# voidful/DeSTA2.5-Audio

Hardware: AMD Instinct MI355X
Metric: train steps/sec (node) Whisper-v3+Llama3.1-8B Q-Former6L at 1/2/4/8 MI355X (higher is better)
Workload: dtype bf16

## Files before the change

desta2.5-audio_amd/csrc/attention.hip:

```cpp
#include "common.h"
#include <mutex>
#include "desta_hip.h"

#ifndef ATTN_ABL
#define ATTN_ABL 0
#endif

namespace {

typedef __attribute__((ext_vector_type(4))) __bf16 bf16x4;

struct AttnArgs {
    const bf16_t* Q; const bf16_t* K; const bf16_t* V; bf16_t* O;
    const bf16_t* dO; bf16_t* dQ; bf16_t* dK; bf16_t* dV;
    float* lse; const float* delta;
    float* O32;
    const float* rope_cs;
    long q_bs, q_rs, k_bs, k_rs, v_bs, v_rs, o_bs, o_rs;
    long do_bs, do_rs, dq_bs, dq_rs, dk_bs, dk_rs, dv_bs, dv_rs;
    int B, Hq, Hkv, Sq, Sk;
    int causal;
    const int* kv_start;
    float scale_log2;
    float scale;
    unsigned drop_thresh, seed_lo, seed_hi; float drop_scale;
    long dkv_t_ld;
};

template <int D>
__device__ __forceinline__ int img_off(int row, int ch) {
    const int sw = (D == 128) ? (((row & 3) << 2) | ((row >> 2) & 3)) : ((((row >> 1) & 1) << 2) | ((row >> 2) & 3));
    return row * (D * 2) + ((ch ^ sw) << 4);
}

template <int N> struct stage_vec;
template <> struct stage_vec<1> { typedef __attribute__((ext_vector_type(4))) unsigned type; };
template <> struct stage_vec<2> { typedef __attribute__((ext_vector_type(8))) unsigned type; };
template <> struct stage_vec<4> { typedef __attribute__((ext_vector_type(16))) unsigned type; };
template <int D, int ROWS, int NT = 256> using stage_t = typename stage_vec<ROWS * (D / 8) / NT>::type;

template <int D, int ROWS, int NT = 256>
__device__ __forceinline__ stage_t<D, ROWS, NT> tile_load(const bf16_t* base, long rs, int row0, int max_row) {
    constexpr int CH = D / 8, N = ROWS * CH / NT;
    stage_t<D, ROWS, NT> out;
#pragma unroll
    for (int i = 0; i < N; ++i) {
        const int id = i * NT + threadIdx.x;
        const int r = id / CH, c = id % CH;
        const int gr = min(row0 + r, max_row);
        const uint4 v = *(const uint4*)(base + (long)gr * rs + c * 8);
        out[4 * i + 0] = v.x; out[4 * i + 1] = v.y; out[4 * i + 2] = v.z; out[4 * i + 3] = v.w;
    }
    return out;
}
template <int D, int ROWS, int NT = 256>
__device__ __forceinline__ void tile_store(char* img, const stage_t<D, ROWS, NT>& regs) {
    constexpr int CH = D / 8, N = ROWS * CH / NT;
#pragma unroll
    for (int i = 0; i < N; ++i) {
        const int id = i * NT + threadIdx.x;
        const int r = id / CH, c = id % CH;
        *(uint4*)(img + img_off<D>(r, c)) = make_uint4(regs[4 * i + 0], regs[4 * i + 1], regs[4 * i + 2], regs[4 * i + 3]);
    }
}

template <int D>
__device__ __forceinline__ bf16x8 frag_rows(const char* img, int row0, int ks, int lane) {
    const int r = row0 + (lane & 31);
    return *(const bf16x8*)(img + img_off<D>(r, 2 * ks + (lane >> 5)));
}

template <int D>
__device__ __forceinline__ bf16x8 frag_tr(const char* img, int row0, int col0, int lane) {
    const int i = lane & 15, g = (lane >> 4) & 1, h = lane >> 5;
    const int q = i >> 2, pp = i & 3;
    const int c = col0 + 16 * g + 4 * pp;
    const int r_lo = row0 + 4 * h + q;
    const int a0 = img_off<D>(r_lo, c >> 3) + ((c & 4) << 1);
    const int a1 = img_off<D>(r_lo + 8, c >> 3) + ((c & 4) << 1);
    const bf16x4 lo = __builtin_amdgcn_ds_read_tr16_b64_v4bf16((__attribute__((address_space(3))) bf16x4*)(img + a0));
    const bf16x4 hi = __builtin_amdgcn_ds_read_tr16_b64_v4bf16((__attribute__((address_space(3))) bf16x4*)(img + a1));
    bf16x8 out;
    out[0] = lo[0]; out[1] = lo[1]; out[2] = lo[2]; out[3] = lo[3];
    out[4] = hi[0]; out[5] = hi[1]; out[6] = hi[2]; out[7] = hi[3];
    return out;
}

__device__ __forceinline__ bf16x8 acc_frag(const f32x16& x, int s) {
    bf16x8 o;
#pragma unroll
    for (int j = 0; j < 8; ++j) o[j] = (__bf16)x[8 * s + j];
    return o;
}

__device__ __forceinline__ int acc_row(int reg, int lane) { return (reg & 3) + 8 * (reg >> 2) + 4 * (lane >> 5); }

__device__ __forceinline__ void attn_work_item(const AttnArgs& p, int nq, int& qblk, int& h, int& b) {
    const int id = blockIdx.x, per = nq * (p.Hq / p.Hkv), ngrp = p.B * p.Hkv;
    int g, r;
    if ((ngrp & 7) == 0) {
        const int xcd = id & 7, slot = id >> 3;
        g = (slot / per) * 8 + xcd;
        r = slot % per;
    } else {
        g = id / per;
        r = id % per;
    }
    b = g / p.Hkv;
    h = (g % p.Hkv) * (p.Hq / p.Hkv) + r / nq;
    qblk = r % nq;
    if (p.causal) qblk = nq - 1 - qblk;
}

#ifndef ATTN_FWD_PF
#define ATTN_FWD_PF 1
#endif
#ifndef ATTN_FWD64_WAVES
#define ATTN_FWD64_WAVES 3
#endif
template <int D, bool DROP, int NW = 4>
__global__ __launch_bounds__(64 * NW, NW == 4 ? (D == 64 ? ATTN_FWD64_WAVES : 2) : 2) void attn_fwd_k(AttnArgs p) {
    constexpr int NT = 64 * NW, QB = 32 * NW;
    __shared__ __attribute__((aligned(16))) char lds[2 * 64 * D * 2];
    char* kimg = lds;
    char* vimg = lds + 64 * D * 2;
    const int lane = threadIdx.x & 63, wave = __builtin_amdgcn_readfirstlane(threadIdx.x >> 6), h2 = lane >> 5;
    int qblk, h, b;
    attn_work_item(p, (p.Sq + QB - 1) / QB, qblk, h, b);
    const int qb0 = qblk * QB, q0 = qb0 + wave * 32;
    const int hk = h / (p.Hq / p.Hkv);
    const int qcol = q0 + (lane & 31);

    const bf16_t* qptr = p.Q + (long)b * p.q_bs + (long)min(qcol, p.Sq - 1) * p.q_rs + (long)h * D;
    bf16x8 qf[D / 16];
#pragma unroll
    for (int ds = 0; ds < D / 16; ++ds) qf[ds] = *(const bf16x8*)(qptr + 16 * ds + 8 * h2);

    const int coff = p.Sk - p.Sq;
    const int kv_lo = p.kv_start ? max(0, min(p.kv_start[b], p.Sk)) : 0;
    int kv_hi = p.Sk;
    if (p.causal) kv_hi = min(p.Sk, min(qb0 + QB - 1, p.Sq - 1) + coff + 1);
    const int t_lo = kv_lo / 64, t_hi = (kv_hi + 63) / 64;
    const int q_abs = qcol + coff;
    const int wave_kmax = p.causal ? min(q0 + 31, p.Sq - 1) + coff : p.Sk - 1;

    const bf16_t* kbase = p.K + (long)b * p.k_bs + (long)hk * D;
    const bf16_t* vbase = p.V + (long)b * p.v_bs + (long)hk * D;

    f32x16 oacc[D / 32];
#pragma unroll
    for (int i = 0; i < D / 32; ++i)
#pragma unroll
        for (int r = 0; r < 16; ++r) oacc[i][r] = 0.f;
    float m = -INFINITY, l = 0.f;

    constexpr int PF = ATTN_FWD_PF;
    stage_t<D, 64, NT> kr0 = {}, vr0 = {}, kr1 = {}, vr1 = {};
    if (t_lo < t_hi) {
        kr0 = tile_load<D, 64, NT>(kbase, p.k_rs, t_lo * 64, p.Sk - 1);
        vr0 = tile_load<D, 64, NT>(vbase, p.v_rs, t_lo * 64, p.Sk - 1);
    }
    if (PF == 2 && t_lo + 1 < t_hi) {
        kr1 = tile_load<D, 64, NT>(kbase, p.k_rs, (t_lo + 1) * 64, p.Sk - 1);
        vr1 = tile_load<D, 64, NT>(vbase, p.v_rs, (t_lo + 1) * 64, p.Sk - 1);
    }
    auto compute = [&](const int kt) __attribute__((always_inline)) {
        if (kt * 64 > wave_kmax) return;
        f32x16 st[2];
#pragma unroll
        for (int kb = 0; kb < 2; ++kb)
#pragma unroll
            for (int r = 0; r < 16; ++r) st[kb][r] = 0.f;
        {
            constexpr int NS = (ATTN_ABL == 4 ? 1 : D / 16);
            bf16x8 ka[NS], kbf[NS];
#pragma unroll
            for (int ds = 0; ds < NS; ++ds) ka[ds] = frag_rows<D>(kimg, 0, ds, lane);
            __builtin_amdgcn_sched_barrier(0);
#pragma unroll
            for (int ds = 0; ds < NS; ++ds) {
                st[0] = __builtin_amdgcn_mfma_f32_32x32x16_bf16(ka[ds], qf[ds], st[0], 0, 0, 0);
                kbf[ds] = frag_rows<D>(kimg, 32, ds, lane);
            }
            __builtin_amdgcn_sched_barrier(0);
#pragma unroll
            for (int ds = 0; ds < NS; ++ds) st[1] = __builtin_amdgcn_mfma_f32_32x32x16_bf16(kbf[ds], qf[ds], st[1], 0, 0, 0);
        }
        const bool need_mask = (kt * 64 + 63 >= p.Sk) || (kt * 64 < kv_lo) || (p.causal && kt * 64 + 63 > q0 + coff);
        if (need_mask) {
            asm volatile("; boundary tile" ::: "memory");
#pragma unroll
            for (int kb = 0; kb < 2; ++kb)
#pragma unroll
                for (int r = 0; r < 16; ++r) {
                    const int key = kt * 64 + kb * 32 + acc_row(r, lane);
                    const bool ok = key < p.Sk && key >= kv_lo && (!p.causal || key <= q_abs);
                    st[kb][r] = ok ? st[kb][r] : -INFINITY;
                }
        }
        float tmax = -INFINITY;
#pragma unroll
        for (int kb = 0; kb < 2; ++kb)
#pragma unroll
            for (int r = 0; r < 16; ++r) tmax = fmaxf(tmax, st[kb][r]);
        tmax = fmaxf(tmax, __shfl_xor(tmax, 32, 64)) * p.scale_log2;
        const float mnew = fmaxf(m, tmax);
        const float muse = (mnew == -INFINITY) ? 0.f : mnew;
        const float alpha = __builtin_amdgcn_exp2f(m - muse);
        typedef float f32x2 __attribute__((ext_vector_type(2)));
        f32x2 rs2 = {0.f, 0.f};
        const f32x2 sc2 = {p.scale_log2, p.scale_log2}, nm2 = {-muse, -muse};
#pragma unroll
        for (int kb = 0; kb < 2; ++kb)
#pragma unroll
            for (int r = 0; r < 16; r += 2) {
                const f32x2 sv = {st[kb][r], st[kb][r + 1]};
                const f32x2 av = sv * sc2 + nm2;
// ... 426 lines not shown
    for (int ds = 0; ds < D / 16; ++ds) {
        qf[ds] = *(const bf16x8*)(qptr + 16 * ds + 8 * h2);
        gf[ds] = *(const bf16x8*)(gptr + 16 * ds + 8 * h2);
    }
    const long stat = ((long)b * p.Hq + h) * p.Sq + qc;
    const float lse = p.lse[stat], dlt = p.delta[stat];

    const int coff = p.Sk - p.Sq;
    const int kv_lo = p.kv_start ? max(0, min(p.kv_start[b], p.Sk)) : 0;
    int kv_hi = p.Sk;
    if (p.causal) kv_hi = min(p.Sk, min(qb0 + QB - 1, p.Sq - 1) + coff + 1);
    const int t_lo = kv_lo / 64, t_hi = (kv_hi + 63) / 64;
    const int q_abs = qcol + coff;
    const int wave_kmax = p.causal ? min(q0 + 31, p.Sq - 1) + coff : p.Sk - 1;

    const bf16_t* kbase = p.K + (long)b * p.k_bs + (long)hk * D;
    const bf16_t* vbase = p.V + (long)b * p.v_bs + (long)hk * D;

    f32x16 dq[D / 32];
#pragma unroll
    for (int i = 0; i < D / 32; ++i)
#pragma unroll
        for (int r = 0; r < 16; ++r) dq[i][r] = 0.f;

    constexpr int PF = ATTN_DQ_PF;
    stage_t<D, 64, NT> kr0 = {}, vr0 = {}, kr1 = {}, vr1 = {};
    if (t_lo < t_hi) {
        kr0 = tile_load<D, 64, NT>(kbase, p.k_rs, t_lo * 64, p.Sk - 1);
        vr0 = tile_load<D, 64, NT>(vbase, p.v_rs, t_lo * 64, p.Sk - 1);
    }
    if (PF == 2 && t_lo + 1 < t_hi) {
        kr1 = tile_load<D, 64, NT>(kbase, p.k_rs, (t_lo + 1) * 64, p.Sk - 1);
        vr1 = tile_load<D, 64, NT>(vbase, p.v_rs, (t_lo + 1) * 64, p.Sk - 1);
    }
    auto compute = [&](const int kt) __attribute__((always_inline)) {
        if (kt * 64 > wave_kmax) return;
#pragma unroll
        for (int kb = 0; kb < 2; ++kb) {
            f32x16 st, dp;
#pragma unroll
            for (int r = 0; r < 16; ++r) { st[r] = 0.f; dp[r] = 0.f; }
#pragma unroll
            for (int ds = 0; ds < D / 16; ++ds) {
                st = __builtin_amdgcn_mfma_f32_32x32x16_bf16(frag_rows<D>(kimg, kb * 32, ds, lane), qf[ds], st, 0, 0, 0);
                dp = __builtin_amdgcn_mfma_f32_32x32x16_bf16(frag_rows<D>(vimg, kb * 32, ds, lane), gf[ds], dp, 0, 0, 0);
            }
            const bool need_mask = (kt * 64 + kb * 32 + 31 >= p.Sk) || (kt * 64 + kb * 32 < kv_lo) ||
                                   (p.causal && kt * 64 + kb * 32 + 31 > q0 + coff);
            unsigned keep = 0xffffu;
            if constexpr (DROP) {
                const unsigned long rowbase = (((unsigned long)b * p.Hq + h) * p.Sq + qc) * p.Sk;
                keep = 0;
#pragma unroll
                for (int r = 0; r < 16; r += 2) {
                    const unsigned long i0 = rowbase + (kt * 64 + kb * 32 + acc_row(r, lane));
                    const unsigned hsh = desta_rng32(p.seed_lo, p.seed_hi, i0 >> 1);
                    keep |= ((hsh & 0xffffu) >= p.drop_thresh ? 1u : 0u) << r;
                    keep |= ((hsh >> 16) >= p.drop_thresh ? 1u : 0u) << (r + 1);
                }
            }
            if (need_mask) {
                asm volatile("; boundary tile" ::: "memory");
#pragma unroll
                for (int r = 0; r < 16; ++r) {
                    const int key = kt * 64 + kb * 32 + acc_row(r, lane);
                    const bool ok = key < p.Sk && key >= kv_lo && (!p.causal || key <= q_abs);
                    st[r] = ok ? st[r] : -INFINITY;
                }
            }
#pragma unroll
            for (int r = 0; r < 16; ++r) {
                const float pv = __builtin_amdgcn_exp2f(fmaf(st[r], p.scale_log2, -lse));
                float dpr = dp[r];
                if constexpr (DROP) dpr = ((keep >> r) & 1u) ? dpr * p.drop_scale : 0.f;
                st[r] = pv * (dpr - dlt) * p.scale;
            }
#pragma unroll
            for (int s = 0; s < 2; ++s) {
                const bf16x8 dsf = acc_frag(st, s);
#pragma unroll
                for (int i = 0; i < D / 32; ++i)
                    dq[i] = __builtin_amdgcn_mfma_f32_32x32x16_bf16(frag_tr<D>(kimg, kb * 32 + 16 * s, i * 32, lane), dsf, dq[i], 0, 0, 0);
            }
        }
    };
#define DESTA_KV_STAGE(KT, KR, VR)                                                   \
    __syncthreads();                         \
    asm volatile("; stage " #KR ::: "memory");  \
    tile_store<D, 64, NT>(kimg, KR);                                                     \
    tile_store<D, 64, NT>(vimg, VR);                                                     \
    __syncthreads();                                                                 \
    if ((KT) + PF < t_hi) {                                                          \
        KR = tile_load<D, 64, NT>(kbase, p.k_rs, ((KT) + PF) * 64, p.Sk - 1);            \
        VR = tile_load<D, 64, NT>(vbase, p.v_rs, ((KT) + PF) * 64, p.Sk - 1);            \
    }
    for (int kt = t_lo; kt < t_hi; kt += 2) {
        DESTA_KV_STAGE(kt, kr0, vr0)
        compute(kt);
        if (kt + 1 < t_hi) {
            if constexpr (PF == 2) {
                DESTA_KV_STAGE(kt + 1, kr1, vr1)
            } else {
                DESTA_KV_STAGE(kt + 1, kr0, vr0)
            }
            compute(kt + 1);
        }
    }
#undef DESTA_KV_STAGE
    if (qcol < p.Sq) {
        bf16_t* optr = p.dQ + (long)b * p.dq_bs + (long)qcol * p.dq_rs + (long)h * D;
#pragma unroll
        for (int i = 0; i < D / 32; ++i)
#pragma unroll
            for (int rq = 0; rq < 4; ++rq) {
                u16x4 o;
#pragma unroll
                for (int e = 0; e < 4; ++e) o[e] = f2bf(dq[i][4 * rq + e]);
                *(u16x4*)(optr + i * 32 + 8 * rq + 4 * h2) = o;
            }
    }
}

template <int D, bool CAUSAL, int HPB>
__global__ __launch_bounds__(512, 2) void attn_bwd_dq8_k(AttnArgs p, float* __restrict__ delta_out) {
    constexpr int NT = 512, RB = 256 / HPB, WPH = RB / 32;
    constexpr int TILE = 64 * D * 2, SLOT = 2 * TILE;
    constexpr int NCH = 64 * (D / 8) / NT;
    __shared__ __attribute__((aligned(16))) char lds[2 * SLOT];
    const int lane = threadIdx.x & 63, wave = __builtin_amdgcn_readfirstlane(threadIdx.x >> 6), h2 = lane >> 5;
    const int G = p.Hq / p.Hkv, nq = (p.Sq + RB - 1) / RB, hgroups = G / HPB, ngrp = p.B * p.Hkv;
    int g, qblk, hg;
    {
        const int id = blockIdx.x, per = nq * hgroups;
        if ((ngrp & 7) == 0) {
            const int xcd = id & 7, slot = id >> 3, gpx = ngrp >> 3;
            if (CAUSAL) {
                const int r = slot % (hgroups * gpx);
                qblk = nq - 1 - slot / (hgroups * gpx); hg = r / gpx; g = (r % gpx) * 8 + xcd;
            } else {
                const int r = slot % per;
                g = (slot / per) * 8 + xcd; hg = r / nq; qblk = r % nq;
            }
        } else if (CAUSAL) {
            const int r = id % (hgroups * ngrp);
            qblk = nq - 1 - id / (hgroups * ngrp); hg = r / ngrp; g = r % ngrp;
        } else {
            const int r = id % per;
            g = id / per; hg = r / nq; qblk = r % nq;
        }
    }
    const int b = g / p.Hkv, hk = g % p.Hkv;
    const int h = hk * G + hg * HPB + wave / WPH;
    const int qb0 = qblk * RB, q0 = qb0 + (wave % WPH) * 32;
    const int qcol = q0 + (lane & 31), qc = min(qcol, p.Sq - 1);
    const bool wave_on = q0 < p.Sq;

    const int coff = p.Sk - p.Sq;
    const int kv_lo = p.kv_start ? max(0, min(p.kv_start[b], p.Sk)) : 0;
    int kv_hi = p.Sk;
    if (CAUSAL) kv_hi = min(p.Sk, min(qb0 + RB - 1, p.Sq - 1) + coff + 1);
    const int t_lo = kv_lo / 64, t_hi = (kv_hi + 63) / 64;
    const int q_abs = qcol + coff;
    const int wave_kmax = CAUSAL ? min(q0 + 31, p.Sq - 1) + coff : p.Sk - 1;

    const char* kbase = (const char*)(p.K + (long)b * p.k_bs + (long)hk * D);
    const char* vbase = (const char*)(p.V + (long)b * p.v_bs + (long)hk * D);
    int srow[NCH], sdst[NCH];
    unsigned ksrc[NCH], vsrc[NCH];
#pragma unroll
    for (int i = 0; i < NCH; ++i) {
        const int id = i * NT + threadIdx.x, r = id / (D / 8), c = id % (D / 8);
        srow[i] = r;
        sdst[i] = img_off<D>(r, c);
        ksrc[i] = (unsigned)(r * (int)p.k_rs + c * 8) * 2u;
        vsrc[i] = (unsigned)(r * (int)p.v_rs + c * 8) * 2u;
    }
    typedef typename stage_vec<NCH>::type stage8_t;
    stage8_t kr = {}, vr = {};
    auto load_tile = [&](const int kt) __attribute__((always_inline)) {
        const char* kb_ = kbase + (long)kt * 64 * p.k_rs * 2;
        const char* vb_ = vbase + (long)kt * 64 * p.v_rs * 2;
        const bool ragged = kt * 64 + 64 > p.Sk;
#pragma unroll
        for (int i = 0; i < NCH; ++i) {
            unsigned ko = ksrc[i], vo = vsrc[i];
            if (ragged) {
                const int rc = max(min(srow[i], p.Sk - 1 - kt * 64), -kt * 64), c = (i * NT + (int)threadIdx.x) % (D / 8);
                ko = (unsigned)(rc * (int)p.k_rs + c * 8) * 2u;
                vo = (unsigned)(rc * (int)p.v_rs + c * 8) * 2u;
            }
            const uint4 a = *(const uint4*)(kb_ + (long)(int)ko), c4 = *(const uint4*)(vb_ + (long)(int)vo);
            kr[4 * i + 0] = a.x; kr[4 * i + 1] = a.y; kr[4 * i + 2] = a.z; kr[4 * i + 3] = a.w;
            vr[4 * i + 0] = c4.x; vr[4 * i + 1] = c4.y; vr[4 * i + 2] = c4.z; vr[4 * i + 3] = c4.w;
        }
    };
    auto store_tile = [&](char* slot) __attribute__((always_inline)) {
#pragma unroll
        for (int i = 0; i < NCH; ++i) {
            *(uint4*)(slot + sdst[i]) = make_uint4(kr[4 * i + 0], kr[4 * i + 1], kr[4 * i + 2], kr[4 * i + 3]);
            *(uint4*)(slot + TILE + sdst[i]) = make_uint4(vr[4 * i + 0], vr[4 * i + 1], vr[4 * i + 2], vr[4 * i + 3]);
        }
    };

    load_tile(t_lo);
    const bf16_t* qptr = p.Q + (long)b * p.q_bs + (long)qc * p.q_rs + (long)h * D;
    const bf16_t* gptr = p.dO + (long)b * p.do_bs + (long)qc * p.do_rs + (long)h * D;
    const bf16_t* optr = p.O + (long)b * p.o_bs + (long)qc * p.o_rs + (long)h * D;
    bf16x8 qf[D / 16], gf[D / 16];
    float dl = 0.f;
#pragma unroll
    for (int ds = 0; ds < D / 16; ++ds) {
        qf[ds] = *(const bf16x8*)(qptr + 16 * ds + 8 * h2);
        gf[ds] = *(const bf16x8*)(gptr + 16 * ds + 8 * h2);
        const bf16x8 of = *(const bf16x8*)(optr + 16 * ds + 8 * h2);
#pragma unroll
        for (int j = 0; j < 8; ++j) dl += (float)of[j] * (float)gf[ds][j];
    }
    const long stat = ((long)b * p.Hq + h) * p.Sq + qc;
    const float nlse = -p.lse[stat];
    const float dlt = swap_halves_sum(dl);
    if (wave_on && qcol < p.Sq && h2 == 0) delta_out[stat] = dlt;
#pragma unroll
    for (int ds = 0; ds < D / 16; ++ds) asm volatile("" :: "v"(qf[ds]), "v"(gf[ds]));
    asm volatile("" :: "v"(nlse));
    store_tile(lds);
    load_tile(t_lo + 1);

    int kofs[D / 16], tofs[D / 32][2];
#pragma unroll
    for (int ds = 0; ds < D / 16; ++ds) {
        kofs[ds] = img_off<D>(lane & 31, 2 * ds + h2);
        asm volatile("" : "+v"(kofs[ds]));
    }
    {
        const int i16 = lane & 15, gq = (lane >> 4) & 1, qq = i16 >> 2, pp = i16 & 3;
#pragma unroll
        for (int i = 0; i < D / 32; ++i) {
            const int c = i * 32 + 16 * gq + 4 * pp;
            tofs[i][0] = img_off<D>(4 * h2 + qq, c >> 3) + ((c & 4) << 1);
            tofs[i][1] = img_off<D>(4 * h2 + qq + 8, c >> 3) + ((c & 4) << 1);
            asm volatile("" : "+v"(tofs[i][0]), "+v"(tofs[i][1]));
        }
    }
    f32x16 dq[D / 32];
#pragma unroll
    for (int i = 0; i < D / 32; ++i)
#pragma unroll
        for (int r = 0; r < 16; ++r) dq[i][r] = 0.f;
#define ATTN_BARRIER() asm volatile("s_waitcnt lgkmcnt(0)\n\ts_barrier" ::: "memory")
    ATTN_BARRIER();

    int sb = 0;
    for (int kt = t_lo; kt < t_hi; ++kt) {
        const int sn = SLOT - sb;
        const bool act = wave_on && kt * 64 <= wave_kmax;
        if (act) {
            int kad[D / 16];
#pragma unroll
            for (int ds = 0; ds < D / 16; ++ds) { kad[ds] = kofs[ds] + sb; asm volatile("" : "+v"(kad[ds])); }
#pragma unroll
            for (int kb = 0; kb < 2; ++kb) {
                if (CAUSAL && kt * 64 + kb * 32 > wave_kmax) break;
                f32x16 st, dp;
#pragma unroll
                for (int r = 0; r < 16; ++r) { st[r] = 0.f; dp[r] = 0.f; }
#pragma unroll
                for (int ds = 0; ds < D / 16; ++ds) {
                    st = __builtin_amdgcn_mfma_f32_32x32x16_bf16(*(const bf16x8*)(lds + kad[ds] + kb * 32 * D * 2), qf[ds], st, 0, 0, 0);
                    dp = __builtin_amdgcn_mfma_f32_32x32x16_bf16(*(const bf16x8*)(lds + kad[ds] + TILE + kb * 32 * D * 2), gf[ds], dp, 0, 0, 0);
                }
                const bool need_mask = (kt * 64 + kb * 32 + 31 >= p.Sk) || (kt * 64 + kb * 32 < kv_lo) ||
                                       (CAUSAL && kt * 64 + kb * 32 + 31 > q0 + coff);
                if (need_mask) {
                    asm volatile("; boundary tile" ::: "memory");
#pragma unroll
                    for (int r = 0; r < 16; ++r) {
                        const int key = kt * 64 + kb * 32 + acc_row(r, lane);
                        const bool ok = key < p.Sk && key >= kv_lo && (!CAUSAL || key <= q_abs);
                        st[r] = ok ? st[r] : -INFINITY;
                    }
                }
#pragma unroll
                for (int r = 0; r < 16; ++r) {
                    const float pv = __builtin_amdgcn_exp2f(fmaf(st[r], p.scale_log2, nlse));
                    st[r] = pv * ((dp[r] - dlt) * p.scale);
                }
                int tad[D / 32][2];
#pragma unroll
                for (int i = 0; i < D / 32; ++i)
#pragma unroll
                    for (int j = 0; j < 2; ++j) { tad[i][j] = tofs[i][j] + sb + kb * 32 * D * 2; asm volatile("" : "+v"(tad[i][j])); }
#pragma unroll
                for (int s = 0; s < 2; ++s) {
                    const bf16x8 dsf = acc_frag(st, s);
#pragma unroll
                    for (int i = 0; i < D / 32; ++i)
                        dq[i] = __builtin_amdgcn_mfma_f32_32x32x16_bf16(tr_pair(lds + tad[i][0] + 16 * s * D * 2, lds + tad[i][1] + 16 * s * D * 2), dsf, dq[i], 0, 0, 0);
                }
            }
        }
        if (kt + 1 < t_hi) {
            store_tile(lds + sn);
            if (kt + 2 < t_hi) load_tile(kt + 2);
        }
        ATTN_BARRIER();
        sb = sn;
    }
#undef ATTN_BARRIER

    if (wave_on && qcol < p.Sq) {
        bf16_t* dqp = p.dQ + (long)b * p.dq_bs + (long)qcol * p.dq_rs + (long)h * D;
        if (p.rope_cs) {
            const float* cs = p.rope_cs + (long)qcol * D;
#pragma unroll
            for (int i = 0; i < D / 32; ++i)
#pragma unroll
                for (int jj = 0; jj < 4; ++jj) {
                    const float4 c4 = *(const float4*)(cs + (32 * i + 8 * jj + 4 * h2));
                    const float g0 = dq[i][4 * jj], g1 = dq[i][4 * jj + 1], g2 = dq[i][4 * jj + 2], g3 = dq[i][4 * jj + 3];
                    dq[i][4 * jj] = g0 * c4.x + g1 * c4.y;     dq[i][4 * jj + 1] = g1 * c4.x - g0 * c4.y;
                    dq[i][4 * jj + 2] = g2 * c4.z + g3 * c4.w; dq[i][4 * jj + 3] = g3 * c4.z - g2 * c4.w;
                }
        }
#pragma unroll
        for (int i = 0; i < D / 32; ++i)
#pragma unroll
            for (int j = 0; j < 2; ++j) {
                unsigned a[2], c[2];
#pragma unroll
                for (int e = 0; e < 2; ++e) {
                    a[e] = (unsigned)f2bf(dq[i][8 * j + 2 * e]) | ((unsigned)f2bf(dq[i][8 * j + 2 * e + 1]) << 16);
                    c[e] = (unsigned)f2bf(dq[i][8 * j + 4 + 2 * e]) | ((unsigned)f2bf(dq[i][8 * j + 4 + 2 * e + 1]) << 16);
                }
                const auto r0 = __builtin_amdgcn_permlane32_swap(a[0], c[0], false, false);
                const auto r1 = __builtin_amdgcn_permlane32_swap(a[1], c[1], false, false);
                *(uint4*)(dqp + i * 32 + 16 * j + 8 * h2) = make_uint4(r0[0], r1[0], r0[1], r1[1]);
            }
    }
}

#ifndef ATTN_DKDV_QR
#define ATTN_DKDV_QR 32
#endif

template <int D, bool DROP, int NW = 4>
__global__ __launch_bounds__(64 * NW, (NW == 4 && D == 64) ? 2 : 1) void attn_bwd_dkdv_k(AttnArgs p) {
    constexpr int QR = (D == 128) ? ATTN_DKDV_QR : 32;
    constexpr int NT = 64 * NW, KB = 32 * NW;
    constexpr int LDS_LOOP = 2 * QR * D * 2 + 2 * QR * 4, LDS_EPI = NW * 32 * 64 * 4;
    __shared__ __attribute__((aligned(16))) char lds[LDS_LOOP > LDS_EPI ? LDS_LOOP : LDS_EPI];
    char* qimg = lds;
    char* gimg = lds + QR * D * 2;
    float* lse_s = (float*)(lds + 2 * QR * D * 2);
    float* dlt_s = lse_s + QR;
    const int lane = threadIdx.x & 63, wave = __builtin_amdgcn_readfirstlane(threadIdx.x >> 6), h2 = lane >> 5;
    const int nhb = p.Hkv * p.B;
    const int kb0 = (blockIdx.x / nhb) * KB, k0 = kb0 + wave * 32;
    const int hk = (blockIdx.x % nhb) % p.Hkv, b = (blockIdx.x % nhb) / p.Hkv, group = p.Hq / p.Hkv;
    const int kcol = k0 + (lane & 31), kc = min(kcol, p.Sk - 1);
    const int kv_lo = p.kv_start ? max(0, min(p.kv_start[b], p.Sk)) : 0;
    const int coff = p.Sk - p.Sq;

    const bf16_t* kptr = p.K + (long)b * p.k_bs + (long)kc * p.k_rs + (long)hk * D;
    const bf16_t* vptr = p.V + (long)b * p.v_bs + (long)kc * p.v_rs + (long)hk * D;
    bf16x8 kf[D / 16], vf[D / 16];
#pragma unroll
    for (int ds = 0; ds < D / 16; ++ds) {
        kf[ds] = *(const bf16x8*)(kptr + 16 * ds + 8 * h2);
        vf[ds] = *(const bf16x8*)(vptr + 16 * ds + 8 * h2);
    }
    const bool key_ok = kcol < p.Sk && kcol >= kv_lo;

    f32x16 dk[D / 32], dv[D / 32];
#pragma unroll
    for (int i = 0; i < D / 32; ++i)
#pragma unroll
        for (int r = 0; r < 16; ++r) { dk[i][r] = 0.f; dv[i][r] = 0.f; }

    const int q_first = p.causal ? max(0, kb0 - coff) : 0;
    const int qt_lo = q_first / QR, qt_hi = (p.Sq + QR - 1) / QR;
    const int nq = qt_hi - qt_lo, n_it = group * nq;
    stage_t<D, QR, NT> qr0 = {}, gr0 = {}, qr1 = {}, gr1 = {};
    float ls0 = 0.f, dl0 = 0.f, ls1 = 0.f, dl1 = 0.f;
#define DESTA_Q_FETCH(IT, QR_, GR, LS, DL)                                                                      \
    {                                                                                                          \
        const int h_ = hk * group + (IT) / nq, qt_ = qt_lo + (IT) % nq;                                        \
        QR_ = tile_load<D, QR, NT>(p.Q + (long)b * p.q_bs + (long)h_ * D, p.q_rs, qt_ * QR, p.Sq - 1);        \
        GR = tile_load<D, QR, NT>(p.dO + (long)b * p.do_bs + (long)h_ * D, p.do_rs, qt_ * QR, p.Sq - 1);      \
        if (threadIdx.x < QR) {                                                                                \
            const long st_ = ((long)b * p.Hq + h_) * p.Sq + min(qt_ * QR + (int)threadIdx.x, p.Sq - 1);       \
            LS = p.lse[st_];                                                                                   \
            DL = p.delta[st_];                                                                                 \
        }                                                                                                      \
    }
#define DESTA_Q_STAGE(IT, QR_, GR, LS, DL)                                                                      \
    __syncthreads();                                                                                           \
    asm volatile("; stage " #QR_ ::: "memory");                                                                \
    tile_store<D, QR, NT>(qimg, QR_);                                                                          \
    tile_store<D, QR, NT>(gimg, GR);                                                                           \
    if (threadIdx.x < QR) { lse_s[threadIdx.x] = LS; dlt_s[threadIdx.x] = DL; }                                \
    __syncthreads();                                                                                           \
    if ((IT) + 2 < n_it) DESTA_Q_FETCH((IT) + 2, QR_, GR, LS, DL)
    if (n_it > 0) DESTA_Q_FETCH(0, qr0, gr0, ls0, dl0)
    if (n_it > 1) DESTA_Q_FETCH(1, qr1, gr1, ls1, dl1)
    auto compute = [&](const int it) __attribute__((always_inline)) {
        const int qt = qt_lo + it % nq;
        constexpr int NS = QR / 32;
        f32x16 stv[NS], dpv[NS];
        bool act[NS];
#pragma unroll
        for (int sub = 0; sub < NS; ++sub) {
            const int qb = qt * QR + sub * 32;
            act[sub] = qb < p.Sq && !(p.causal && k0 > qb + 31 + coff);
            if (!act[sub]) continue;
#pragma unroll
            for (int r = 0; r < 16; ++r) { stv[sub][r] = 0.f; dpv[sub][r] = 0.f; }
#pragma unroll
            for (int ds = 0; ds < D / 16; ++ds) {
                stv[sub] = __builtin_amdgcn_mfma_f32_32x32x16_bf16(frag_rows<D>(qimg, sub * 32, ds, lane), kf[ds], stv[sub], 0, 0, 0);
                dpv[sub] = __builtin_amdgcn_mfma_f32_32x32x16_bf16(frag_rows<D>(gimg, sub * 32, ds, lane), vf[ds], dpv[sub], 0, 0, 0);
            }
        }
#pragma unroll
        for (int sub = 0; sub < NS; ++sub) {
            if (!act[sub]) continue;
            const int qb = qt * QR + sub * 32;
            f32x16& st = stv[sub];
            f32x16& dp = dpv[sub];
            const bool need_mask = (qb + 31 >= p.Sq) || (k0 + 31 >= p.Sk) || (k0 < kv_lo) ||
                                   (p.causal && k0 + 31 > qb + coff);
            float lsv[16], dlv[16];
#pragma unroll
            for (int q4 = 0; q4 < 4; ++q4) {
                const float4 a4 = *(const float4*)(lse_s + sub * 32 + 8 * q4 + 4 * h2);
                const float4 b4 = *(const float4*)(dlt_s + sub * 32 + 8 * q4 + 4 * h2);
                lsv[4 * q4 + 0] = a4.x; lsv[4 * q4 + 1] = a4.y; lsv[4 * q4 + 2] = a4.z; lsv[4 * q4 + 3] = a4.w;
                dlv[4 * q4 + 0] = b4.x; dlv[4 * q4 + 1] = b4.y; dlv[4 * q4 + 2] = b4.z; dlv[4 * q4 + 3] = b4.w;
            }
            unsigned keep = 0xffffu;
            if constexpr (DROP) {
                const unsigned long hb = ((unsigned long)b * p.Hq + (hk * group + it / nq)) * p.Sq;
                keep = 0;
                const int half = lane & 1, kpair = k0 + (lane & 30);
                unsigned hh[8];
#pragma unroll
                for (int j = 0; j < 8; ++j) {
                    const int ql = (j & 3) + 8 * (2 * half + (j >> 2)) + 4 * h2;
                    hh[j] = desta_rng32(p.seed_lo, p.seed_hi, ((hb + min(qb + ql, p.Sq - 1)) * p.Sk + kpair) >> 1);
                }
#pragma unroll
                for (int j = 0; j < 8; ++j) {
                    const unsigned oth = (unsigned)__builtin_amdgcn_mov_dpp((int)hh[j], 0xB1, 0xf, 0xf, true);
                    const unsigned mine = half ? (hh[j] >> 16) : (hh[j] & 0xffffu), theirs = half ? (oth >> 16) : (oth & 0xffffu);
                    keep |= (mine >= p.drop_thresh ? 1u : 0u) << (8 * half + j);
                    keep |= (theirs >= p.drop_thresh ? 1u : 0u) << (8 * (1 - half) + j);
                }
            }
            if (need_mask) {
                asm volatile("; boundary slice" ::: "memory");
#pragma unroll
                for (int r = 0; r < 16; ++r) {
                    const int q = qb + acc_row(r, lane);
                    const bool ok = key_ok && q < p.Sq && (!p.causal || kcol <= q + coff);
                    st[r] = ok ? st[r] : -INFINITY;
                }
            }
#pragma unroll
            for (int r = 0; r < 16; ++r) {
                const float pv = __builtin_amdgcn_exp2f(fmaf(st[r], p.scale_log2, -lsv[r]));
                float ms = 1.0f;
                if constexpr (DROP) ms = ((keep >> r) & 1u) ? p.drop_scale : 0.f;
                st[r] = pv * ms;
                dp[r] = pv * (ms * dp[r] - dlv[r]) * p.scale;
            }
#pragma unroll
            for (int s = 0; s < 2; ++s) {
                const bf16x8 pf = acc_frag(st, s), dsf = acc_frag(dp, s);
#pragma unroll
                for (int i = 0; i < D / 32; ++i) {
                    dv[i] = __builtin_amdgcn_mfma_f32_32x32x16_bf16(pf, frag_tr<D>(gimg, sub * 32 + 16 * s, i * 32, lane), dv[i], 0, 0, 0);
                    dk[i] = __builtin_amdgcn_mfma_f32_32x32x16_bf16(dsf, frag_tr<D>(qimg, sub * 32 + 16 * s, i * 32, lane), dk[i], 0, 0, 0);
                }
            }
        }
    };
    for (int it = 0; it < n_it; it += 2) {
        DESTA_Q_STAGE(it, qr0, gr0, ls0, dl0)
        compute(it);
        if (it + 1 < n_it) {
            DESTA_Q_STAGE(it + 1, qr1, gr1, ls1, dl1)
            compute(it + 1);
        }
    }
#undef DESTA_Q_STAGE
#undef DESTA_Q_FETCH
    bf16_t* dkp = p.dK + (long)b * p.dk_bs + (long)hk * D;
    bf16_t* dvp = p.dV + (long)b * p.dv_bs + (long)hk * D;
    const bool wide = ((p.dk_rs | p.dv_rs | p.dk_bs | p.dv_bs) & 7) == 0 && (((size_t)p.dK | (size_t)p.dV) & 15) == 0;
    if (wide) {
        __syncthreads();
        float* tb = (float*)lds + wave * (32 * 64);
        auto emit = [&](const f32x16 (&acc)[D / 32], bf16_t* base, long rs, const bool rope) __attribute__((always_inline)) {
#pragma unroll
            for (int hf = 0; hf < D / 64; ++hf) {
#pragma unroll
                for (int ii = 0; ii < 2; ++ii)
#pragma unroll
                    for (int r = 0; r < 16; ++r) tb[acc_row(r, lane) * 64 + ii * 32 + (lane & 31)] = acc[hf * 2 + ii][r];
                asm volatile("s_waitcnt lgkmcnt(0)" ::: "memory");
#pragma unroll
                for (int j = 0; j < 4; ++j) {
                    const int row = (lane >> 3) + 8 * j, key = k0 + row;
                    float4 x0 = *(const float4*)(tb + row * 64 + (lane & 7) * 8), x1 = *(const float4*)(tb + row * 64 + (lane & 7) * 8 + 4);
                    if (rope) {
                        const float* cs = p.rope_cs + (long)min(key, p.Sk - 1) * D + hf * 64 + (lane & 7) * 8;
                        const float4 c0 = *(const float4*)cs, c1 = *(const float4*)(cs + 4);
                        const float4 y0 = make_float4(x0.x * c0.x + x0.y * c0.y, x0.y * c0.x - x0.x * c0.y, x0.z * c0.z + x0.w * c0.w, x0.w * c0.z - x0.z * c0.w);
                        const float4 y1 = make_float4(x1.x * c1.x + x1.y * c1.y, x1.y * c1.x - x1.x * c1.y, x1.z * c1.z + x1.w * c1.w, x1.w * c1.z - x1.z * c1.w);
                        x0 = y0; x1 = y1;
                    }
                    u16x8 o;
                    o[0] = f2bf(x0.x); o[1] = f2bf(x0.y); o[2] = f2bf(x0.z); o[3] = f2bf(x0.w);
                    o[4] = f2bf(x1.x); o[5] = f2bf(x1.y); o[6] = f2bf(x1.z); o[7] = f2bf(x1.w);
                    if (key < p.Sk) *(u16x8*)(base + (long)key * rs + hf * 64 + (lane & 7) * 8) = o;
                }
                asm volatile("s_waitcnt lgkmcnt(0)" ::: "memory");
            }
        };
        emit(dk, dkp, p.dk_rs, p.rope_cs != nullptr);
        emit(dv, dvp, p.dv_rs, false);
        return;
    }
#pragma unroll
    for (int i = 0; i < D / 32; ++i)
#pragma unroll
        for (int r = 0; r < 16; ++r) {
            const int key = k0 + acc_row(r, lane);
            if (key < p.Sk) {
                dkp[(long)key * p.dk_rs + i * 32 + (lane & 31)] = f2bf(dk[i][r]);
                dvp[(long)key * p.dv_rs + i * 32 + (lane & 31)] = f2bf(dv[i][r]);
            }
        }
}

template <bool DROP, bool TR>
__global__ __launch_bounds__(256, 2) void attn_bwd_q64_k(AttnArgs p, float* __restrict__ dq_part, float* __restrict__ bias_part, int blocks_per_chunk) {
    constexpr int D = 64, WREG = 12288;
    __shared__ __attribute__((aligned(16))) char lds[2 * 64 * D * 2 + 4 * WREG + 2 * 64 * 4];
    char* qimg = lds;
    char* gimg = lds + 64 * D * 2;
    char* wreg = lds + 2 * 64 * D * 2;
    float* lse_s = (float*)(wreg + 4 * WREG);
    float* dlt_s = lse_s + 64;
    const int lane = threadIdx.x & 63, wave = __builtin_amdgcn_readfirstlane(threadIdx.x >> 6), h2 = lane >> 5;
    const int nbh = p.B * p.Hq;
    const int chunk = blockIdx.x / nbh, bh = blockIdx.x % nbh, b = bh / p.Hq, h = bh % p.Hq;
    const int nkb = (p.Sk + 127) / 128;
    const int kb_lo = chunk * blocks_per_chunk, kb_hi = min(kb_lo + blocks_per_chunk, nkb);
    const int kv_lo = p.kv_start ? max(0, min(p.kv_start[b], p.Sk)) : 0;
    char* kimg_w = wreg + wave * WREG;
    char* vimg_w = kimg_w + 4096;
    char* dsimg_w = kimg_w + 8192;
    const bf16_t* kbase = p.K + (long)b * p.k_bs + (long)h * D;
    const bf16_t* vbase = p.V + (long)b * p.v_bs + (long)h * D;

    {
        const stage_t<D, 64> qr = tile_load<D, 64>(p.Q + (long)b * p.q_bs + (long)h * D, p.q_rs, 0, p.Sq - 1);
        const stage_t<D, 64> gr = tile_load<D, 64>(p.dO + (long)b * p.do_bs + (long)h * D, p.do_rs, 0, p.Sq - 1);
        tile_store<D, 64>(qimg, qr);
        tile_store<D, 64>(gimg, gr);
        if (threadIdx.x < 64) {
            const long st_ = ((long)b * p.Hq + h) * p.Sq + min((int)threadIdx.x, p.Sq - 1);
            lse_s[threadIdx.x] = p.lse[st_];
            dlt_s[threadIdx.x] = p.delta[st_];
        }
    }
    const int qa = wave >> 1, di = wave & 1;
    f32x16 dq;
#pragma unroll
    for (int r = 0; r < 16; ++r) dq[r] = 0.f;

    stage_t<D, 128> kst = {}, vst = {};
    if (kb_lo < kb_hi) {
        kst = tile_load<D, 128>(kbase, p.k_rs, kb_lo * 128, p.Sk - 1);
        vst = tile_load<D, 128>(vbase, p.v_rs, kb_lo * 128, p.Sk - 1);
    }
    const unsigned long hb = ((unsigned long)b * p.Hq + h) * p.Sq;
    bf16_t* dkp = TR ? p.dK + (long)h * D * p.dkv_t_ld + (long)b * p.Sk : p.dK + (long)b * p.dk_bs + (long)h * D;
    bf16_t* dvp = TR ? p.dV + (long)h * D * p.dkv_t_ld + (long)b * p.Sk : p.dV + (long)b * p.dv_bs + (long)h * D;
    float bsum[2][2] = {{0.f, 0.f}, {0.f, 0.f}};

    for (int kb = kb_lo; kb < kb_hi; ++kb) {
        __syncthreads();
#pragma unroll
        for (int i = 0; i < 4; ++i) {
            const int id = i * 256 + threadIdx.x, r = id >> 3, c = id & 7;
            char* dst = wreg + (r >> 5) * WREG + img_off<D>(r & 31, c);
            *(uint4*)dst = make_uint4(kst[4 * i + 0], kst[4 * i + 1], kst[4 * i + 2], kst[4 * i + 3]);
            *(uint4*)(dst + 4096) = make_uint4(vst[4 * i + 0], vst[4 * i + 1], vst[4 * i + 2], vst[4 * i + 3]);
        }
        __syncthreads();
        if (kb + 1 < kb_hi) {
            kst = tile_load<D, 128>(kbase, p.k_rs, (kb + 1) * 128, p.Sk - 1);
            vst = tile_load<D, 128>(vbase, p.v_rs, (kb + 1) * 128, p.Sk - 1);
        }
        const int k0 = kb * 128 + wave * 32, kcol = k0 + (lane & 31);
        const bool key_ok = kcol < p.Sk && kcol >= kv_lo;
        f32x16 dk[2], dv[2];
#pragma unroll
        for (int i = 0; i < 2; ++i)
#pragma unroll
            for (int r = 0; r < 16; ++r) { dk[i][r] = 0.f; dv[i][r] = 0.f; }
#pragma unroll 1
        for (int sub = 0; sub < 2; ++sub) {
            const int qb = sub * 32;
            if (qb >= p.Sq) {
#pragma unroll
                for (int j = 0; j < 4; ++j) *(uint2*)(dsimg_w + img_off<D>(lane & 31, sub * 4 + j) + 8 * h2) = make_uint2(0u, 0u);
                continue;
            }
            unsigned keep = 0xffffu;
            if constexpr (DROP) {
                keep = 0;
                const int half = lane & 1, kpair = k0 + (lane & 30);
                unsigned hh[8];
                const unsigned long e0 = (hb + qb) * p.Sk + kpair;
#pragma unroll
                for (int j = 0; j < 8; ++j) {
                    const int ql = (j & 3) + 8 * (2 * half + (j >> 2)) + 4 * h2;
                    hh[j] = desta_rng32(p.seed_lo, p.seed_hi, (e0 + (unsigned)(ql * p.Sk)) >> 1);
                }
#pragma unroll
                for (int j = 0; j < 8; ++j) {
                    const unsigned oth = (unsigned)__builtin_amdgcn_mov_dpp((int)hh[j], 0xB1, 0xf, 0xf, true);
                    const unsigned mine = half ? (hh[j] >> 16) : (hh[j] & 0xffffu), theirs = half ? (oth >> 16) : (oth & 0xffffu);
                    keep |= (mine >= p.drop_thresh ? 1u : 0u) << (8 * half + j);
                    keep |= (theirs >= p.drop_thresh ? 1u : 0u) << (8 * (1 - half) + j);
                }
            }
            if constexpr (DROP) asm volatile("" : "+v"(keep));
            f32x16 st, dp;
#pragma unroll
            for (int r = 0; r < 16; ++r) { st[r] = 0.f; dp[r] = 0.f; }
#pragma unroll
            for (int ds = 0; ds < D / 16; ++ds) {
                st = __builtin_amdgcn_mfma_f32_32x32x16_bf16(frag_rows<D>(qimg, qb, ds, lane), frag_rows<D>(kimg_w, 0, ds, lane), st, 0, 0, 0);
                dp = __builtin_amdgcn_mfma_f32_32x32x16_bf16(frag_rows<D>(gimg, qb, ds, lane), frag_rows<D>(vimg_w, 0, ds, lane), dp, 0, 0, 0);
            }
            const bool need_mask = (qb + 31 >= p.Sq) || (k0 + 31 >= p.Sk) || (k0 < kv_lo);
            if (need_mask) {
#pragma unroll
                for (int r = 0; r < 16; ++r) {
                    const bool ok = key_ok && (qb + acc_row(r, lane)) < p.Sq;
                    st[r] = ok ? st[r] : -INFINITY;
                }
            }
#pragma unroll
            for (int q4 = 0; q4 < 4; ++q4) {
                const float4 a4 = *(const float4*)(lse_s + qb + 8 * q4 + 4 * h2);
                const float4 b4 = *(const float4*)(dlt_s + qb + 8 * q4 + 4 * h2);
                const float ls4[4] = {a4.x, a4.y, a4.z, a4.w}, dl4[4] = {b4.x, b4.y, b4.z, b4.w};
#pragma unroll
                for (int e = 0; e < 4; ++e) {
                    const int r = 4 * q4 + e;
                    const float pv = __builtin_amdgcn_exp2f(fmaf(st[r], p.scale_log2, -ls4[e]));
                    float ms = 1.0f;
                    if constexpr (DROP) ms = ((keep >> r) & 1u) ? p.drop_scale : 0.f;
                    st[r] = pv * ms;
                    dp[r] = pv * (ms * dp[r] - dl4[e]) * p.scale;
                }
            }
#pragma unroll
            for (int j = 0; j < 4; ++j) {
                const unsigned lo = (unsigned)f2bf(dp[4 * j + 0]) | ((unsigned)f2bf(dp[4 * j + 1]) << 16);
                const unsigned hi = (unsigned)f2bf(dp[4 * j + 2]) | ((unsigned)f2bf(dp[4 * j + 3]) << 16);
                *(uint2*)(dsimg_w + img_off<D>(lane & 31, sub * 4 + j) + 8 * h2) = make_uint2(lo, hi);
            }
#pragma unroll
            for (int s2 = 0; s2 < 2; ++s2) {
                const bf16x8 pf = acc_frag(st, s2), dsf = acc_frag(dp, s2);
#pragma unroll
                for (int i = 0; i < 2; ++i) {
                    dv[i] = __builtin_amdgcn_mfma_f32_32x32x16_bf16(pf, frag_tr<D>(gimg, qb + 16 * s2, i * 32, lane), dv[i], 0, 0, 0);
                    dk[i] = __builtin_amdgcn_mfma_f32_32x32x16_bf16(dsf, frag_tr<D>(qimg, qb + 16 * s2, i * 32, lane), dk[i], 0, 0, 0);
                }
            }
        }
        __syncthreads();
#pragma unroll
        for (int wv = 0; wv < 4; ++wv)
#pragma unroll
            for (int s2 = 0; s2 < 2; ++s2)
                dq = __builtin_amdgcn_mfma_f32_32x32x16_bf16(frag_tr<D>(wreg + wv * WREG + 8192, 16 * s2, qa * 32, lane),
// ... 399 lines not shown
    f32x4 st[NT16];
    float mx = -INFINITY;
#pragma unroll
    for (int t = 0; t < NT16; ++t) {
        st[t] = f32x4{0.f, 0.f, 0.f, 0.f};
#pragma unroll
        for (int ks = 0; ks < 4; ++ks) st[t] = __builtin_amdgcn_mfma_f32_16x16x32_bf16(e4m3x8_to_bf16(kq[t][ks]), qf[ks], st[t], 0, 0, 0);
#pragma unroll
        for (int r = 0; r < 4; ++r) {
            const int key = k0 + 16 * t + 4 * q4 + r;
            st[t][r] = (key >= kv_lo && key < p.Sk) ? (st[t][r] * ksc[t][r]) * p.scale_log2 : -INFINITY;
            mx = fmaxf(mx, st[t][r]);
        }
    }
    mx = fmaxf(mx, __shfl_xor(mx, 16, 64));
    mx = fmaxf(mx, __shfl_xor(mx, 32, 64));
    if (lane < 8) s_m[wave][lane] = mx;
    __syncthreads();
    const int g8 = c16 & 7;
    const float mblk = fmaxf(fmaxf(s_m[0][g8], s_m[1][g8]), fmaxf(s_m[2][g8], s_m[3][g8]));
    const float muse = (mblk == -INFINITY) ? 0.f : mblk;
    float ls = 0.f;
#pragma unroll
    for (int t = 0; t < NT16; ++t)
#pragma unroll
        for (int r = 0; r < 4; ++r) {
            const float pv = __builtin_amdgcn_exp2f(st[t][r] - muse);
            ls += pv;
            if (c16 < 8) s_p[wave][16 * t + 4 * q4 + r][c16] = pv * vsc[t][r];
        }
    ls += __shfl_xor(ls, 16, 64);
    ls += __shfl_xor(ls, 32, 64);
    if (lane < 8) s_l[wave][lane] = ls;
    __syncthreads();

    float acc[GP][8];
#pragma unroll
    for (int g = 0; g < GP; ++g)
#pragma unroll
        for (int j = 0; j < 8; ++j) acc[g][j] = 0.f;
#pragma unroll
    for (int i = 0; i < NV; ++i) {
        const float* pr = &s_p[wave][4 * i + q4][0];
        float pg[GP];
        if constexpr (GP >= 4) {
#pragma unroll
            for (int g = 0; g < GP; g += 4) {
                const f32x4 t4 = *(const f32x4*)(pr + g);
                pg[g] = t4[0]; pg[g + 1] = t4[1]; pg[g + 2] = t4[2]; pg[g + 3] = t4[3];
            }
        } else {
#pragma unroll
            for (int g = 0; g < GP; ++g) pg[g] = pr[g];
        }
        const f32x2 vv[4] = {__builtin_amdgcn_cvt_pk_f32_fp8((int)vq[i].x, false), __builtin_amdgcn_cvt_pk_f32_fp8((int)vq[i].x, true),
                             __builtin_amdgcn_cvt_pk_f32_fp8((int)vq[i].y, false), __builtin_amdgcn_cvt_pk_f32_fp8((int)vq[i].y, true)};
#pragma unroll
        for (int j2 = 0; j2 < 4; ++j2) {
            const float v0 = vv[j2][0], v1 = vv[j2][1];
#pragma unroll
            for (int g = 0; g < GP; ++g) {
                acc[g][2 * j2] = fmaf(pg[g], v0, acc[g][2 * j2]);
                acc[g][2 * j2 + 1] = fmaf(pg[g], v1, acc[g][2 * j2 + 1]);
            }
        }
    }
    const bool hi32 = (lane & 32) != 0, hi16 = (lane & 16) != 0;
    constexpr int G1 = GP >= 2 ? GP / 2 : GP, G2 = GP >= 4 ? GP / 4 : G1;
    float a1[G1][8], a2[G2][8];
#pragma unroll
    for (int g = 0; g < G1; ++g)
#pragma unroll
        for (int j = 0; j < 8; ++j) {
            if constexpr (GP >= 2) {
                const float keep = hi32 ? acc[g + G1][j] : acc[g][j], send = hi32 ? acc[g][j] : acc[g + G1][j];
                a1[g][j] = keep + __shfl_xor(send, 32, 64);
            } else {
                a1[g][j] = acc[g][j] + __shfl_xor(acc[g][j], 32, 64);
            }
        }
#pragma unroll
    for (int g = 0; g < G2; ++g)
#pragma unroll
        for (int j = 0; j < 8; ++j) {
            if constexpr (GP >= 4) {
                const float keep = hi16 ? a1[g + G2][j] : a1[g][j], send = hi16 ? a1[g][j] : a1[g + G2][j];
                a2[g][j] = keep + __shfl_xor(send, 16, 64);
            } else {
                a2[g][j] = a1[g][j] + __shfl_xor(a1[g][j], 16, 64);
            }
        }
    {
        const int gbase = (GP >= 2 && hi32 ? G1 : 0) + (GP >= 4 && hi16 ? G2 : 0);
        const bool writer = GP >= 4 ? true : (GP == 2 ? !hi16 : lane < 16);
        if (writer)
#pragma unroll
            for (int g = 0; g < G2; ++g) {
                float* dst = &s_red[wave][gbase + g][8 * c16];
                *(f32x4*)dst = f32x4{a2[g][0], a2[g][1], a2[g][2], a2[g][3]};
                *(f32x4*)(dst + 4) = f32x4{a2[g][4], a2[g][5], a2[g][6], a2[g][7]};
            }
    }
    __syncthreads();

    const int tg = threadIdx.x >> 5, d4 = threadIdx.x & 31;
    if (tg < G) {
        f32x4 o = *(const f32x4*)&s_red[0][tg][4 * d4];
#pragma unroll
        for (int w = 1; w < 4; ++w) o += *(const f32x4*)&s_red[w][tg][4 * d4];
        const float m = fmaxf(fmaxf(s_m[0][tg], s_m[1][tg]), fmaxf(s_m[2][tg], s_m[3][tg]));
        const float l = ((s_l[0][tg] + s_l[1][tg]) + s_l[2][tg]) + s_l[3][tg];
        const int h = hk * G + tg;
        if (nch == 1) {
            u16x4 ob;
#pragma unroll
            for (int e = 0; e < 4; ++e) ob[e] = f2bf(l > 0.f ? o[e] / l : 0.f);
            *(u16x4*)(p.O + (long)b * p.o_bs + (long)h * 128 + 4 * d4) = ob;
            if (p.lse && d4 == 0) p.lse[(long)b * p.Hq + h] = l > 0.f ? m + log2f(l) : INFINITY;
        } else {
            const long r = ((long)b * p.Hq + h) * nch + c;
            *(f32x4*)(ws_o + r * 128 + 4 * d4) = o;
            if (d4 == 0) { ws_ml[2 * r] = m; ws_ml[2 * r + 1] = l; }
        }
    }
}

int fill_args(const desta_attn_desc* d, AttnArgs& a) {
    DESTA_CHECK_ARG(d && d->Q && d->K && d->V, "attention: null operand");
    DESTA_CHECK_ARG(d->head_dim == 64 || d->head_dim == 128, "attention: head_dim %d unsupported (64 or 128)", d->head_dim);
    DESTA_CHECK_ARG(d->batch > 0 && d->n_q_heads > 0 && d->n_kv_heads > 0 && d->n_q_heads % d->n_kv_heads == 0,
                    "attention: bad head counts");
    DESTA_CHECK_ARG(d->seq_q > 0 && d->seq_k > 0, "attention: bad sequence lengths");
    DESTA_CHECK_ARG(!d->causal || d->seq_k >= d->seq_q, "attention: causal needs seq_k >= seq_q");
    DESTA_CHECK_ARG(d->q_row_stride % 8 == 0 && d->k_row_stride % 8 == 0 && d->v_row_stride % 8 == 0,
                    "attention: row strides must be multiples of 8 elements");
    DESTA_CHECK_ARG(d->batch <= 65535 && d->n_q_heads <= 65535, "attention: grid too large");
    a.Q = (const bf16_t*)d->Q; a.K = (const bf16_t*)d->K; a.V = (const bf16_t*)d->V; a.O = (bf16_t*)d->O;
    a.dO = (const bf16_t*)d->dO; a.dQ = (bf16_t*)d->dQ; a.dK = (bf16_t*)d->dK; a.dV = (bf16_t*)d->dV;
    a.lse = d->lse; a.delta = nullptr; a.O32 = d->O_f32; a.rope_cs = d->rope_cos_sin;
    a.q_bs = d->q_batch_stride; a.q_rs = d->q_row_stride; a.k_bs = d->k_batch_stride; a.k_rs = d->k_row_stride;
    a.v_bs = d->v_batch_stride; a.v_rs = d->v_row_stride; a.o_bs = d->o_batch_stride; a.o_rs = d->o_row_stride;
    a.do_bs = d->do_batch_stride; a.do_rs = d->do_row_stride; a.dq_bs = d->dq_batch_stride; a.dq_rs = d->dq_row_stride;
    a.dk_bs = d->dk_batch_stride; a.dk_rs = d->dk_row_stride; a.dv_bs = d->dv_batch_stride; a.dv_rs = d->dv_row_stride;
    a.B = d->batch; a.Hq = d->n_q_heads; a.Hkv = d->n_kv_heads; a.Sq = d->seq_q; a.Sk = d->seq_k;
    a.causal = d->causal; a.kv_start = d->kv_start;
    a.scale = d->scale; a.scale_log2 = d->scale * 1.44269504088896340736f;
    DESTA_CHECK_ARG(d->dropout_p >= 0.f && d->dropout_p < 1.f, "attention: dropout_p must be in [0,1)");
    DESTA_CHECK_ARG(d->dropout_p == 0.f || d->head_dim == 64, "attention: dropout is built for head_dim 64 (the Q-Former) only");
    DESTA_CHECK_ARG(d->dropout_p == 0.f || d->seq_k % 2 == 0, "attention: dropout needs an even seq_k (adjacent keys share one hash)");
    a.drop_thresh = d->dropout_p > 0.f ? desta_drop_thresh(d->dropout_p) : 0u;
    a.drop_scale = 1.0f / (1.0f - d->dropout_p);
    a.seed_lo = (unsigned)d->dropout_seed; a.seed_hi = (unsigned)(d->dropout_seed >> 32);
    a.dkv_t_ld = d->dkv_transposed ? d->dkv_t_ld : 0;
    return DESTA_OK;
}

}

namespace { int g_attn_opt[8] = {1, 0, 0, 0, 1, 0, 0, 0}; }
extern "C" int desta_attention_set_option(int which, int value) {
    DESTA_CHECK_ARG(which >= 0 && which < 8, "attention_set_option: unknown option %d", which);
    g_attn_opt[which] = value;
    return DESTA_OK;
}

extern "C" int desta_attention_fwd(const desta_attn_desc* d, void* stream) {
    AttnArgs a;
    if (int rc = fill_args(d, a)) return rc;
    DESTA_CHECK_ARG(d->O, "attention_fwd: null output");
    DESTA_CHECK_ARG(d->o_row_stride % 8 == 0 && d->o_batch_stride % 8 == 0 && ((size_t)d->O & 15) == 0,
                    "attention_fwd: O must be 16-byte aligned with row / batch strides that are multiples of 8 elements");
    if (g_attn_opt[0] && !a.drop_thresh && a.Sq >= 128) {
        const int G = a.Hq / a.Hkv;
        const int hpb = !a.causal ? 1 : (d->head_dim == 128 ? (G % 4 == 0 ? 4 : (G % 2 == 0 ? 2 : 1)) : (G % 2 == 0 ? 2 : 1));
        const int rb = 256 / hpb;
        dim3 g8((unsigned)((a.Sq + rb - 1) / rb) * (unsigned)(G / hpb) * (unsigned)(a.B * a.Hkv));
        hipStream_t st = (hipStream_t)stream;
        if (d->head_dim == 128) {
            if (!a.causal) hipLaunchKernelGGL((attn_fwd8_k<128, false, 1>), g8, dim3(512), 0, st, a);
            else if (hpb == 4 && g_attn_opt[2]) hipLaunchKernelGGL((attn_fwd8_k<128, true, 4, 2, true>), g8, dim3(512), 0, st, a);
            else if (hpb == 4) hipLaunchKernelGGL((attn_fwd8_k<128, true, 4>), g8, dim3(512), 0, st, a);
            else if (hpb == 2) hipLaunchKernelGGL((attn_fwd8_k<128, true, 2>), g8, dim3(512), 0, st, a);
            else hipLaunchKernelGGL((attn_fwd8_k<128, true, 1>), g8, dim3(512), 0, st, a);
        } else {
            if (!a.causal && g_attn_opt[1]) hipLaunchKernelGGL((attn_fwd8_k<64, false, 1, 4, false>), g8, dim3(512), 0, st, a);
            else if (!a.causal && g_attn_opt[2]) hipLaunchKernelGGL((attn_fwd8_k<64, false, 1, 2, true>), g8, dim3(512), 0, st, a);
            else if (!a.causal) hipLaunchKernelGGL((attn_fwd8_k<64, false, 1>), g8, dim3(512), 0, st, a);
            else if (hpb == 2) hipLaunchKernelGGL((attn_fwd8_k<64, true, 2>), g8, dim3(512), 0, st, a);
            else hipLaunchKernelGGL((attn_fwd8_k<64, true, 1>), g8, dim3(512), 0, st, a);
        }
        DESTA_CHECK_LAUNCH("attention_fwd");
        return DESTA_OK;
    }
    const bool two = d->head_dim == 64 && a.Sq <= 64;
    dim3 grid((unsigned)((a.Sq + (two ? 63 : 127)) / (two ? 64 : 128)) * a.Hq * a.B);
    if (d->head_dim == 128) hipLaunchKernelGGL((attn_fwd_k<128, false>), grid, dim3(256), 0, (hipStream_t)stream, a);
    else if (two && a.drop_thresh) hipLaunchKernelGGL((attn_fwd_k<64, true, 2>), grid, dim3(128), 0, (hipStream_t)stream, a);
    else if (two) hipLaunchKernelGGL((attn_fwd_k<64, false, 2>), grid, dim3(128), 0, (hipStream_t)stream, a);
    else if (a.drop_thresh) hipLaunchKernelGGL((attn_fwd_k<64, true>), grid, dim3(256), 0, (hipStream_t)stream, a);
    else hipLaunchKernelGGL((attn_fwd_k<64, false>), grid, dim3(256), 0, (hipStream_t)stream, a);
    DESTA_CHECK_LAUNCH("attention_fwd");
    return DESTA_OK;
}

static_assert(DESTA_ATTN_DECODE_CHUNK % 64 == 0 && DESTA_ATTN_DECODE_CHUNK >= 64, "the decode chunk is a multiple of 64 keys");
namespace {
inline size_t decode_ml_floats(size_t items) { return (2 * items + 3) / 4 * 4; }
}
extern "C" int desta_attention_decode_chunk(void) { return DESTA_ATTN_DECODE_CHUNK; }
extern "C" size_t desta_attention_decode_workspace_bytes(int batch, int n_q_heads, int seq_k, int head_dim) {
    if (batch <= 0 || n_q_heads <= 0 || seq_k <= DESTA_ATTN_DECODE_CHUNK || head_dim <= 0) return 0;
    const size_t nch = ((size_t)seq_k + DESTA_ATTN_DECODE_CHUNK - 1) / DESTA_ATTN_DECODE_CHUNK;
    const size_t items = (size_t)batch * n_q_heads * nch;
    return (decode_ml_floats(items) + items * (size_t)head_dim) * sizeof(float);
}

extern "C" int desta_attention_decode(const desta_attn_desc* d, void* workspace, size_t workspace_bytes, void* stream) {
    DESTA_CHECK_ARG(d, "attention_decode: null descriptor");
    DESTA_CHECK_ARG(d->seq_q == 1, "attention_decode: seq_q %d unsupported (one query row per sequence)", d->seq_q);
    DESTA_CHECK_ARG(d->head_dim == 128, "attention_decode: head_dim %d unsupported (128)", d->head_dim);
    DESTA_CHECK_ARG(!d->causal, "attention_decode: causal must be 0 (the one query row sees every key of [kv_start, seq_k))");
    DESTA_CHECK_ARG(d->dropout_p == 0.f, "attention_decode: dropout_p must be 0");
    DESTA_CHECK_ARG(!d->rope_cos_sin, "attention_decode: rope_cos_sin must be NULL");
    DESTA_CHECK_ARG(!d->O_f32, "attention_decode: O_f32 must be NULL");
    DESTA_CHECK_ARG(!d->dO && !d->dQ, "attention_decode: dO and dQ must be NULL (forward only)");
    AttnArgs a;
    if (int rc = fill_args(d, a)) return rc;
    const int G = a.Hq / a.Hkv;
    DESTA_CHECK_ARG(G <= 8, "attention_decode: group of %d query heads per kv head unsupported (at most 8)", G);
    DESTA_CHECK_ARG(d->O && ((size_t)d->O & 15) == 0 && d->o_batch_stride % 8 == 0,
                    "attention_decode: O must be 16-byte aligned with a batch stride that is a multiple of 8 elements");
    DESTA_CHECK_ARG((((size_t)d->Q | (size_t)d->K | (size_t)d->V) & 15) == 0 && d->q_batch_stride % 8 == 0 &&
                    d->k_batch_stride % 8 == 0 && d->v_batch_stride % 8 == 0,
                    "attention_decode: Q, K, V must be 16-byte aligned with batch strides that are multiples of 8 elements");
    const int nch = (a.Sk + DESTA_ATTN_DECODE_CHUNK - 1) / DESTA_ATTN_DECODE_CHUNK;
    const size_t need = desta_attention_decode_workspace_bytes(a.B, a.Hq, a.Sk, 128);
    DESTA_CHECK_ARG(need == 0 || (workspace && workspace_bytes >= need && ((size_t)workspace & 15) == 0),
                    "attention_decode: workspace of %zu bytes is too small or misaligned (%zu needed, 16-byte aligned)", workspace_bytes, need);
    DESTA_CHECK_ARG((long)a.B * a.Hkv * nch <= 0x7fffffffL, "attention_decode: grid too large");
    float* ws_ml = (float*)workspace;
    float* ws_o = ws_ml ? ws_ml + decode_ml_floats((size_t)a.B * a.Hq * nch) : nullptr;
    const dim3 grid((unsigned)(a.B * a.Hkv * nch));
    hipStream_t st = (hipStream_t)stream;
    if (G == 1) hipLaunchKernelGGL((attn_decode_k<1>), grid, dim3(256), 0, st, a, ws_ml, ws_o, nch);
    else if (G == 2) hipLaunchKernelGGL((attn_decode_k<2>), grid, dim3(256), 0, st, a, ws_ml, ws_o, nch);
    else if (G <= 4) hipLaunchKernelGGL((attn_decode_k<4>), grid, dim3(256), 0, st, a, ws_ml, ws_o, nch);
    else hipLaunchKernelGGL((attn_decode_k<8>), grid, dim3(256), 0, st, a, ws_ml, ws_o, nch);
    DESTA_CHECK_LAUNCH("attention_decode");
    if (nch > 1) {
        hipLaunchKernelGGL(attn_decode_combine_k, dim3((unsigned)((a.B * a.Hq + 7) / 8)), dim3(256), 0, st, a, ws_ml, ws_o, nch);
        DESTA_CHECK_LAUNCH("attention_decode (combine)");
    }
    return DESTA_OK;
}

extern "C" int desta_attention_decode_kv8(const desta_attn_desc* d, const float* k_scale, const float* v_scale, int64_t scale_batch_stride,
                                          int64_t scale_row_stride, void* workspace, size_t workspace_bytes, void* stream) {
    DESTA_CHECK_ARG(d, "attention_decode_kv8: null descriptor");
    DESTA_CHECK_ARG(k_scale && v_scale && scale_batch_stride >= 0 && scale_row_stride > 0, "attention_decode_kv8: null scale or bad scale stride");
    DESTA_CHECK_ARG(d->seq_q == 1, "attention_decode_kv8: seq_q %d unsupported (one query row per sequence)", d->seq_q);
    DESTA_CHECK_ARG(d->head_dim == 128, "attention_decode_kv8: head_dim %d unsupported (128)", d->head_dim);
    DESTA_CHECK_ARG(!d->causal, "attention_decode_kv8: causal must be 0 (the one query row sees every key of [kv_start, seq_k))");
    DESTA_CHECK_ARG(d->dropout_p == 0.f, "attention_decode_kv8: dropout_p must be 0");
    DESTA_CHECK_ARG(!d->rope_cos_sin, "attention_decode_kv8: rope_cos_sin must be NULL");
    DESTA_CHECK_ARG(!d->O_f32, "attention_decode_kv8: O_f32 must be NULL");
    DESTA_CHECK_ARG(!d->dO && !d->dQ, "attention_decode_kv8: dO and dQ must be NULL (forward only)");
    AttnArgs a;
    if (int rc = fill_args(d, a)) return rc;
    const int G = a.Hq / a.Hkv;
    DESTA_CHECK_ARG(G <= 8, "attention_decode_kv8: group of %d query heads per kv head unsupported (at most 8)", G);
    DESTA_CHECK_ARG(d->O && ((size_t)d->O & 15) == 0 && d->o_batch_stride % 8 == 0,
                    "attention_decode_kv8: O must be 16-byte aligned with a batch stride that is a multiple of 8 elements");
    DESTA_CHECK_ARG((((size_t)d->Q | (size_t)d->K | (size_t)d->V) & 15) == 0 && d->q_batch_stride % 8 == 0 &&
                    d->k_batch_stride % 8 == 0 && d->v_batch_stride % 8 == 0,
                    "attention_decode_kv8: Q, K, V must be 16-byte aligned with batch strides that are multiples of 8 elements");
    const int nch = (a.Sk + DESTA_ATTN_DECODE_CHUNK - 1) / DESTA_ATTN_DECODE_CHUNK;
    const size_t need = desta_attention_decode_workspace_bytes(a.B, a.Hq, a.Sk, 128);
    DESTA_CHECK_ARG(need == 0 || (workspace && workspace_bytes >= need && ((size_t)workspace & 15) == 0),
                    "attention_decode_kv8: workspace of %zu bytes is too small or misaligned (%zu needed, 16-byte aligned)", workspace_bytes, need);
    DESTA_CHECK_ARG((long)a.B * a.Hkv * nch <= 0x7fffffffL, "attention_decode_kv8: grid too large");
    float* ws_ml = (float*)workspace;
    float* ws_o = ws_ml ? ws_ml + decode_ml_floats((size_t)a.B * a.Hq * nch) : nullptr;
    const dim3 grid((unsigned)(a.B * a.Hkv * nch));
    hipStream_t st = (hipStream_t)stream;
    const long sbs = (long)scale_batch_stride, srs = (long)scale_row_stride;
    if (G == 1) hipLaunchKernelGGL((attn_kv8_k<1>), grid, dim3(256), 0, st, a, k_scale, v_scale, sbs, srs, ws_ml, ws_o, nch);
    else if (G == 2) hipLaunchKernelGGL((attn_kv8_k<2>), grid, dim3(256), 0, st, a, k_scale, v_scale, sbs, srs, ws_ml, ws_o, nch);
    else if (G <= 4) hipLaunchKernelGGL((attn_kv8_k<4>), grid, dim3(256), 0, st, a, k_scale, v_scale, sbs, srs, ws_ml, ws_o, nch);
    else hipLaunchKernelGGL((attn_kv8_k<8>), grid, dim3(256), 0, st, a, k_scale, v_scale, sbs, srs, ws_ml, ws_o, nch);
    DESTA_CHECK_LAUNCH("attention_decode_kv8");
    if (nch > 1) {
        hipLaunchKernelGGL(attn_decode_combine_k, dim3((unsigned)((a.B * a.Hq + 7) / 8)), dim3(256), 0, st, a, ws_ml, ws_o, nch);
        DESTA_CHECK_LAUNCH("attention_decode_kv8 (combine)");
    }
    return DESTA_OK;
}

namespace {
constexpr int KV8_DQ_SLOTS = 16;
__global__ __launch_bounds__(256) void kv8_dequant_k(const uint8_t* __restrict__ cache, long c_bs, long c_rs, const float* __restrict__ scale,
                                                     long s_bs, long s_rs, const int* __restrict__ kv_start, int n_heads, int slot1,
                                                     bf16_t* __restrict__ out, long o_bs, long o_rs) {
    const int b = blockIdx.y;
    const int kv_lo = kv_start ? max(0, min(kv_start[b], slot1)) : 0;
    const int first = max((int)blockIdx.x * KV8_DQ_SLOTS, kv_lo), last = min((int)blockIdx.x * KV8_DQ_SLOTS + KV8_DQ_SLOTS, slot1);
    if (first >= last) return;
    const int per = n_heads * 8;
    const int items = (last - first) * per;
    cache += (long)b * c_bs;
    scale += (long)b * s_bs;
    out += (long)b * o_bs;
    for (int i = threadIdx.x; i < items; i += 256) {
        const int s = first + i / per, r = i % per;
        const uint4 q = *(const uint4*)(cache + (long)s * c_rs + 16 * r);
        const float sc = scale[(long)s * s_rs + (r >> 3)];
        union { bf16x8 v; u16x8 u; } lo, hi;
        lo.v = e4m3x8_to_bf16(make_uint2(q.x, q.y));
        hi.v = e4m3x8_to_bf16(make_uint2(q.z, q.w));
#pragma unroll
        for (int e = 0; e < 8; ++e) {
            lo.u[e] = f2bf(bf2f(lo.u[e]) * sc);
            hi.u[e] = f2bf(bf2f(hi.u[e]) * sc);
        }
        bf16_t* o = out + (long)s * o_rs + 16 * r;
        *(u16x8*)o = lo.u;
        *(u16x8*)(o + 8) = hi.u;
    }
}
}

extern "C" int desta_kv8_dequant(const uint8_t* kv_cache, int64_t kv_batch_stride, int64_t kv_row_stride, const float* kv_scale,
                                 int64_t scale_batch_stride, int64_t scale_row_stride, const int32_t* kv_start, int batch, int n_heads,
                                 int head_dim, int slot1, void* out_bf16, int64_t out_batch_stride, int64_t out_row_stride, void* stream) {
    DESTA_CHECK_ARG(kv_cache && kv_scale && out_bf16, "kv8_dequant: null cache, scale or output");
    DESTA_CHECK_ARG(head_dim == 128, "kv8_dequant: head_dim %d unsupported (128)", head_dim);
    DESTA_CHECK_ARG(batch > 0 && batch <= 65535 && n_heads > 0 && n_heads <= 4096, "kv8_dequant: bad batch %d or n_heads %d", batch, n_heads);
    DESTA_CHECK_ARG(slot1 > 0, "kv8_dequant: slot1 %d must be positive", slot1);
    const long w = (long)n_heads * 128;
    DESTA_CHECK_ARG(((size_t)kv_cache & 15) == 0 && kv_row_stride >= w && kv_row_stride % 16 == 0 && kv_batch_stride >= 0 && kv_batch_stride % 16 == 0,
                    "kv8_dequant: cache must be 16-byte aligned with row / batch strides that are multiples of 16 bytes, rows of at least %ld", w);
    DESTA_CHECK_ARG(scale_row_stride >= n_heads && scale_batch_stride >= 0, "kv8_dequant: bad scale stride");
    DESTA_CHECK_ARG(((size_t)out_bf16 & 15) == 0 && out_row_stride >= w && out_row_stride % 8 == 0 && out_batch_stride >= 0 && out_batch_stride % 8 == 0,
                    "kv8_dequant: output must be 16-byte aligned with row / batch strides that are multiples of 8 elements, rows of at least %ld", w);
    const dim3 grid((unsigned)((slot1 + KV8_DQ_SLOTS - 1) / KV8_DQ_SLOTS), (unsigned)batch);
    hipLaunchKernelGGL(kv8_dequant_k, grid, dim3(256), 0, (hipStream_t)stream, kv_cache, (long)kv_batch_stride, (long)kv_row_stride, kv_scale,
                       (long)scale_batch_stride, (long)scale_row_stride, (const int*)kv_start, n_heads, slot1, (bf16_t*)out_bf16,
                       (long)out_batch_stride, (long)out_row_stride);
    DESTA_CHECK_LAUNCH("kv8_dequant");
    return DESTA_OK;
}

#define ATTN_Q64_MAX_CHUNKS 4
extern "C" size_t desta_attention_bwd_workspace_floats(int batch, int n_q_heads, int seq_q) {
    const size_t delta = ((size_t)batch * n_q_heads * seq_q + 3) / 4 * 4;
    return delta + (seq_q <= 64 ? (size_t)ATTN_Q64_MAX_CHUNKS * batch * n_q_heads * (4096 + 128) : 0);
}

namespace {
struct BwdFork { hipStream_t side = nullptr; hipEvent_t fork = nullptr, join = nullptr; int handles = 0; };
BwdFork g_bwd_fork[16];
std::mutex g_bwd_fork_mu;
int g_bwd_concurrent = 1;
BwdFork* bwd_fork_locked(int dev) {
    BwdFork& f = g_bwd_fork[dev];
    if (!f.side) {
        hipStream_t s = nullptr; hipEvent_t e0 = nullptr, e1 = nullptr;
        if (hipStreamCreateWithFlags(&s, hipStreamNonBlocking) != hipSuccess) return nullptr;
        if (hipEventCreateWithFlags(&e0, hipEventDisableTiming) != hipSuccess ||
            hipEventCreateWithFlags(&e1, hipEventDisableTiming) != hipSuccess) {
            if (e0) (void)hipEventDestroy(e0);
            (void)hipStreamDestroy(s);
            return nullptr;
        }
        f.fork = e0; f.join = e1; f.side = s;
    }
    return &f;
}
BwdFork* bwd_fork() {
    int dev = 0;
    if (hipGetDevice(&dev) != hipSuccess || dev < 0 || dev >= 16) return nullptr;
    if (g_bwd_fork[dev].side) return &g_bwd_fork[dev];
    std::lock_guard<std::mutex> lk(g_bwd_fork_mu);
    return bwd_fork_locked(dev);
}
}
extern "C" int desta_attention_set_concurrent_bwd(int on) { g_bwd_concurrent = on; return DESTA_OK; }
int desta_internal_reserve(void) {
    int dev = 0;
    if (hipGetDevice(&dev) != hipSuccess || dev < 0 || dev >= 16) return DESTA_EINVAL;
    std::lock_guard<std::mutex> lk(g_bwd_fork_mu);
    BwdFork* f = bwd_fork_locked(dev);
    if (!f) return DESTA_ELAUNCH;
    ++f->handles;
    return DESTA_OK;
}
int desta_internal_release(void) {
    int dev = 0;
    if (hipGetDevice(&dev) != hipSuccess || dev < 0 || dev >= 16) return DESTA_EINVAL;
    std::lock_guard<std::mutex> lk(g_bwd_fork_mu);
    BwdFork& f = g_bwd_fork[dev];
    if (f.handles > 0 && --f.handles > 0) return DESTA_OK;
    if (f.side) { (void)hipStreamSynchronize(f.side); (void)hipStreamDestroy(f.side); }
    if (f.fork) (void)hipEventDestroy(f.fork);
    if (f.join) (void)hipEventDestroy(f.join);
    f = BwdFork();
    return DESTA_OK;
}

extern "C" int desta_attention_bwd(const desta_attn_desc* d, float* workspace, void* stream) {
    AttnArgs a;
    if (int rc = fill_args(d, a)) return rc;
    DESTA_CHECK_ARG(d->O && d->dO && d->lse && workspace && d->dQ, "attention_bwd: null argument");
    DESTA_CHECK_ARG((d->dK == nullptr) == (d->dV == nullptr), "attention_bwd: dK and dV go together");
    DESTA_CHECK_ARG(d->dq_row_stride % 4 == 0 && d->do_row_stride % 8 == 0 && d->o_row_stride % 8 == 0,
                    "attention_bwd: bad strides");
    a.delta = workspace;
    hipStream_t st = (hipStream_t)stream;
    const long rows = (long)a.B * a.Hq * a.Sq;
    const int G = d->head_dim / 8;
    dim3 gd((unsigned)((rows * G + 255) / 256));
    dim3 gk_((unsigned)((a.Sk + 127) / 128) * a.Hkv * a.B);
    if (a.rope_cs)
        DESTA_CHECK_ARG(g_attn_opt[0] && !g_attn_opt[3] && !a.drop_thresh && !a.O32 && a.Sq >= 128 && a.Sq == a.Sk && d->dq_row_stride % 8 == 0 &&
                        d->dq_batch_stride % 8 == 0 && ((size_t)d->dQ & 15) == 0 &&
                        (!d->dK || ((((d->dk_row_stride | d->dv_row_stride | d->dk_batch_stride | d->dv_batch_stride) & 7) == 0) &&
                                    (((size_t)d->dK | (size_t)d->dV) & 15) == 0)),
                        "attention_bwd: rope_cos_sin needs seq_q == seq_k >= 128, no dropout and 16-byte aligned dQ / dK / dV");
    if (g_attn_opt[0] && !g_attn_opt[3] && !a.drop_thresh && !a.O32 && a.Sq >= 128 && d->dq_row_stride % 8 == 0 && d->dq_batch_stride % 8 == 0 &&
        ((size_t)d->dQ & 15) == 0) {
        const int G = a.Hq / a.Hkv;
        const int hpb = !a.causal ? 1 : (d->head_dim == 128 ? (G % 4 == 0 ? 4 : (G % 2 == 0 ? 2 : 1)) : (G % 2 == 0 ? 2 : 1));
        const int rb = 256 / hpb;
        dim3 g8((unsigned)((a.Sq + rb - 1) / rb) * (unsigned)(G / hpb) * (unsigned)(a.B * a.Hkv));
        if (d->head_dim == 128) {
            if (!a.causal) hipLaunchKernelGGL((attn_bwd_dq8_k<128, false, 1>), g8, dim3(512), 0, st, a, workspace);
            else if (hpb == 4) hipLaunchKernelGGL((attn_bwd_dq8_k<128, true, 4>), g8, dim3(512), 0, st, a, workspace);
            else if (hpb == 2) hipLaunchKernelGGL((attn_bwd_dq8_k<128, true, 2>), g8, dim3(512), 0, st, a, workspace);
            else hipLaunchKernelGGL((attn_bwd_dq8_k<128, true, 1>), g8, dim3(512), 0, st, a, workspace);
            if (d->dK) {
                if (g_attn_opt[5] && a.causal) {
                    dim3 gk2((unsigned)((a.Sk + 63) / 64) * a.Hkv * a.B);
                    hipLaunchKernelGGL((attn_bwd_dkdv_k<128, false, 2>), gk2, dim3(128), 0, st, a);
                } else hipLaunchKernelGGL((attn_bwd_dkdv_k<128, false>), gk_, dim3(256), 0, st, a);
            }
        } else {
            if (!a.causal) hipLaunchKernelGGL((attn_bwd_dq8_k<64, false, 1>), g8, dim3(512), 0, st, a, workspace);
            else if (hpb == 2) hipLaunchKernelGGL((attn_bwd_dq8_k<64, true, 2>), g8, dim3(512), 0, st, a, workspace);
            else hipLaunchKernelGGL((attn_bwd_dq8_k<64, true, 1>), g8, dim3(512), 0, st, a, workspace);
            if (d->dK) hipLaunchKernelGGL((attn_bwd_dkdv_k<64, false>), gk_, dim3(256), 0, st, a);
        }
        DESTA_CHECK_LAUNCH("attention_bwd");
        return DESTA_OK;
    }
    const bool q64 = d->head_dim == 64 && a.Sq <= 64 && a.Sk >= 256 && !a.causal && a.Hq == a.Hkv && d->dK && !a.rope_cs &&
                     ((d->q_batch_stride | d->k_batch_stride | d->v_batch_stride | d->do_batch_stride) & 7) == 0 && ((size_t)d->dO & 15) == 0 &&
                     (d->dq_batch_stride & 3) == 0 && ((size_t)d->dQ & 7) == 0;
    if (d->dkv_transposed)
        DESTA_CHECK_ARG(q64 && a.Sk % 4 == 0 && d->dkv_t_ld % 4 == 0 && d->dkv_t_ld >= (int64_t)a.B * a.Sk && (((size_t)d->dK | (size_t)d->dV) & 7) == 0,
                        "attention_bwd: dkv_transposed needs the one-query-tile path (head_dim 64, seq_q <= 64, seq_k >= 256 and a multiple of 4, no GQA) and 8-byte aligned dK / dV");
    if ((g_attn_opt[4] || d->dkv_transposed) && q64 &&
        (d->dkv_transposed || (((d->dk_row_stride | d->dv_row_stride | d->dk_batch_stride | d->dv_batch_stride) & 7) == 0 && (((size_t)d->dK | (size_t)d->dV) & 15) == 0))) {
        hipLaunchKernelGGL(attn_delta_k<64>, gd, dim3(256), 0, st, a, workspace);
        const int nkb = (a.Sk + 127) / 128;
        const int nch = nkb >= 8 ? ATTN_Q64_MAX_CHUNKS : (nkb >= 4 ? 2 : 1), bpc = (nkb + nch - 1) / nch;
        float* part = workspace + (rows + 3) / 4 * 4;
        float* bpart = d->dkv_bias_grad ? part + (size_t)ATTN_Q64_MAX_CHUNKS * a.B * a.Hq * 4096 : nullptr;
        dim3 gf((unsigned)(nch * a.B * a.Hq));
        if (d->dkv_transposed) {
            if (a.drop_thresh) hipLaunchKernelGGL((attn_bwd_q64_k<true, true>), gf, dim3(256), 0, st, a, part, bpart, bpc);
            else hipLaunchKernelGGL((attn_bwd_q64_k<false, true>), gf, dim3(256), 0, st, a, part, bpart, bpc);
            if (bpart) hipLaunchKernelGGL(attn_bias_sum_k, dim3((unsigned)(2 * a.Hq)), dim3(256), 0, st, (const float*)bpart,
                                          nch * a.B, 2 * a.Hq * 64, d->dkv_bias_grad);
        } else if (a.drop_thresh) hipLaunchKernelGGL((attn_bwd_q64_k<true, false>), gf, dim3(256), 0, st, a, part, bpart, bpc);
        else hipLaunchKernelGGL((attn_bwd_q64_k<false, false>), gf, dim3(256), 0, st, a, part, bpart, bpc);
        hipLaunchKernelGGL(attn_dq_sum_k, dim3((unsigned)(a.B * a.Hq)), dim3(256), 0, st, a, (const float*)part, nch);
        DESTA_CHECK_LAUNCH("attention_bwd");
        return DESTA_OK;
    }
    const bool two_q = d->head_dim == 64 && a.Sq <= 64;
    dim3 gq((unsigned)((a.Sq + (two_q ? 63 : 127)) / (two_q ? 64 : 128)) * a.Hq * a.B);
    dim3 gk((unsigned)((a.Sk + 127) / 128) * a.Hkv * a.B);
    if (d->head_dim == 128) {
        hipLaunchKernelGGL(attn_delta_k<128>, gd, dim3(256), 0, st, a, workspace);
        BwdFork* f = (g_bwd_concurrent && d->dK) ? bwd_fork() : nullptr;
        if (f && hipEventRecord(f->fork, st) == hipSuccess && hipStreamWaitEvent(f->side, f->fork, 0) == hipSuccess) {
            hipLaunchKernelGGL((attn_bwd_dkdv_k<128, false>), gk, dim3(256), 0, st, a);
            hipLaunchKernelGGL((attn_bwd_dq_k<128, false>), gq, dim3(256), 0, f->side, a);
            DESTA_CHECK_ARG(hipEventRecord(f->join, f->side) == hipSuccess && hipStreamWaitEvent(st, f->join, 0) == hipSuccess,
                            "attention_bwd: could not join the side stream");
        } else {
            hipLaunchKernelGGL((attn_bwd_dq_k<128, false>), gq, dim3(256), 0, st, a);
            if (d->dK) hipLaunchKernelGGL((attn_bwd_dkdv_k<128, false>), gk, dim3(256), 0, st, a);
        }
    } else {
        hipLaunchKernelGGL(attn_delta_k<64>, gd, dim3(256), 0, st, a, workspace);
        const bool two = two_q;
        if (a.drop_thresh) {
            if (two) hipLaunchKernelGGL((attn_bwd_dq_k<64, true, 2>), gq, dim3(128), 0, st, a);
            else hipLaunchKernelGGL((attn_bwd_dq_k<64, true>), gq, dim3(256), 0, st, a);
            if (d->dK) hipLaunchKernelGGL((attn_bwd_dkdv_k<64, true>), gk, dim3(256), 0, st, a);
        } else {
            if (two) hipLaunchKernelGGL((attn_bwd_dq_k<64, false, 2>), gq, dim3(128), 0, st, a);
            else hipLaunchKernelGGL((attn_bwd_dq_k<64, false>), gq, dim3(256), 0, st, a);
            if (d->dK) hipLaunchKernelGGL((attn_bwd_dkdv_k<64, false>), gk, dim3(256), 0, st, a);
        }
    }
    DESTA_CHECK_LAUNCH("attention_bwd");
    return DESTA_OK;
}
```

desta2.5-audio_amd/desta/_hip.py:

```python
from __future__ import annotations

import ctypes as C
import os

import torch

_HERE = os.path.dirname(os.path.abspath(__file__))
LIB_PATH = os.environ.get("DESTA_HIP_LIB") or os.path.join(_HERE, "lib", "libdesta_hip.so")

if not os.path.exists(LIB_PATH):
    raise ImportError(
        f"{LIB_PATH} is missing: build it with `python desta2.5-audio_amd/build.py` "
        "(hipcc --offload-arch=gfx950). There is no CPU/eager fallback for the DeSTA2.5 hot path.")

lib = C.CDLL(LIB_PATH, mode=C.RTLD_GLOBAL)

vp, i32, i64, f32 = C.c_void_p, C.c_int, C.c_int64, C.c_float


class GemmDesc(C.Structure):
    _fields_ = [("A", vp), ("B", vp), ("C", vp),
                ("M", i32), ("N", i32), ("K", i32), ("batch", i32),
                ("lda", i64), ("ldb", i64), ("ldc", i64),
                ("stride_a", i64), ("stride_b", i64), ("stride_c", i64),
# ... 300 lines not shown
_add = _sig("desta_add_f32", vp, vp, i64, vp)
_transpose = _sig("desta_transpose_to_bf16", vp, i32, i64, i32, i32, vp, i64, vp)
_mel_rows = _sig("desta_mel_to_rows", vp, i32, i32, i32, i32, vp, vp)

_scratch = {}


def scratch(nfloats: int, device, tag="ws") -> torch.Tensor:
    key = (str(device), tag)
    t = _scratch.get(key)
    if t is None or t.numel() < nfloats:
        t = torch.empty(max(nfloats, 1024), dtype=torch.float32, device=device)
        _scratch[key] = t
    return t


@_profiled("layernorm_fwd", lambda x, g, b, eps, y16=None, y32=None, stats=None: x.numel() * (x.element_size() + (2 if y16 is not None else 0) + (4 if y32 is not None else 0)))
def layernorm_fwd(x, gamma, beta, eps, y16=None, y32=None, stats=None):
    rows, cols = x.numel() // x.shape[-1], x.shape[-1]
    check(_ln_fwd(p(x), int(x.dtype == torch.float32), p(gamma), p(beta), eps, rows, cols, p(y16), p(y32), p(stats),
                  stream()), "desta_layernorm_fwd")


@_profiled("layernorm_bwd", lambda dy, x, g, st, dx32=None, dx16=None, **k: x.numel() * (dy.element_size() + x.element_size() + (4 if dx32 is not None else 0) + (2 if dx16 is not None else 0)))
def layernorm_bwd(dy, x, gamma, stats, dx32=None, dx16=None, dgamma=None, dbeta=None, accumulate=False):
    rows, cols = x.numel() // x.shape[-1], x.shape[-1]
    ws = scratch(lib.desta_layernorm_bwd_workspace_floats(rows, cols), x.device) if dgamma is not None else None
    check(_ln_bwd(p(dy), int(dy.dtype == torch.float32), p(x), int(x.dtype == torch.float32), p(gamma), p(stats), rows,
                  cols, p(dx32), p(dx16), p(dgamma), p(dbeta), int(accumulate), p(ws), stream()), "desta_layernorm_bwd")


@_profiled("rmsnorm_fwd", lambda x, w, eps, y, rstd=None: 4 * x.numel())
def rmsnorm_fwd(x, weight, eps, y, rstd=None):
    rows, cols = x.numel() // x.shape[-1], x.shape[-1]
    check(_rms_fwd(p(x), p(weight), eps, rows, cols, p(y), p(rstd), stream()), "desta_rmsnorm_fwd")


@_profiled("rmsnorm_bwd", lambda dy, x, w, rstd, dx, dres=None: x.numel() * (6 + (2 if dres is not None else 0)))
def rmsnorm_bwd(dy, x, weight, rstd, dx, dres=None):
    rows, cols = x.numel() // x.shape[-1], x.shape[-1]
    check(_rms_bwd(p(dy), p(x), p(weight), p(rstd), p(dres), rows, cols, p(dx), stream()), "desta_rmsnorm_bwd")


def colsum(x, rows, cols, ld, out, accumulate=False, tag="ws"):
    ws = scratch(lib.desta_colsum_workspace_floats(rows, cols), x.device, tag)
    check(_colsum(p(x), rows, cols, ld, p(out), int(accumulate), p(ws), stream()), "desta_colsum_bf16")


@_profiled("rope", lambda buf, ld, rows, seq, n_q, n_kv, hd, *a, **k: 4 * rows * (n_q + n_kv) * hd)
def rope(buf, ld, rows, seq, n_q, n_kv, hd, cos_sin, q_norm_w=None, k_norm_w=None, eps=1e-6, pre_norm=None,
         ld_pre=0, backward=False, pos_shift=None, s_major_batch=0):
    check(_rope(p(buf), ld, rows, seq, n_q, n_kv, hd, p(cos_sin), p(q_norm_w), p(k_norm_w), eps, p(pre_norm), ld_pre,
                int(backward), p(pos_shift), s_major_batch, stream()), "desta_rope")


@_profiled("swiglu_fwd", lambda gu, act, rows, inter: 6 * rows * inter)
def swiglu_fwd(gate_up, act, rows, inter):
    check(_swiglu_fwd(p(gate_up), p(act), rows, inter, stream()), "desta_swiglu_fwd")


@_profiled("swiglu_bwd", lambda gu, dact, dgu, rows, inter: 10 * rows * inter)
def swiglu_bwd(gate_up, dact, dgate_up, rows, inter):
    check(_swiglu_bwd(p(gate_up), p(dact), p(dgate_up), rows, inter, stream()), "desta_swiglu_bwd")


def gelu_bwd(preact, dact, dpre, n):
    check(_gelu_bwd(p(preact), p(dact), p(dpre), n, stream()), "desta_gelu_bwd")


def cast_bf16(x, y, n=None):
    check(_cast(p(x), p(y), x.numel() if n is None else n, stream()), "desta_cast_f32_bf16")


def add_f32(y, x, n=None):
    check(_add(p(y), p(x), y.numel() if n is None else n, stream()), "desta_add_f32")


def transpose_to_bf16(src, rows, cols, out, ld_out, ld_in=None):
    check(_transpose(p(src), int(src.dtype == torch.float32), cols if ld_in is None else ld_in, rows, cols, p(out),
                     ld_out, stream()), "desta_transpose_to_bf16")


def mel_to_rows(mel, c_pad, out):
    B, Cn, T = mel.shape
    check(_mel_rows(p(mel), B, Cn, T, c_pad, p(out), stream()), "desta_mel_to_rows")


_embed = _sig("desta_embed_gather", vp, vp, vp, i32, i32, vp, vp)
_gather = _sig("desta_gather_rows_bf16", vp, vp, i32, i32, vp, vp)
lib.desta_ce_workspace_floats.restype = c_size_t
lib.desta_ce_workspace_floats.argtypes = [i32, i32]
_ce = _sig("desta_causal_lm_loss", vp, i64, vp, i32, i32, i32, vp, vp, i32, vp)
_token_logprobs = _sig("desta_token_logprobs", vp, i64, vp, i32, i32, vp, vp, vp)
_topk_logprobs = _sig("desta_topk_logprobs", vp, i64, vp, i32, i32, i32, vp, vp, vp, vp)
TOPK_LOGPROBS_MAX = 32
TOPK_LOGPROBS_CALLS = 0
_mix_fwd = _sig("desta_tap_mix_fwd", vp, vp, i32, i32, i32, i32, vp, vp)
_mix_bwd = _sig("desta_tap_mix_bwd", vp, vp, vp, i32, i32, i32, i32, vp, vp, vp)


def embed_gather(table, audio_rows, src_row, rows, hidden, out):
    check(_embed(p(table), p(audio_rows), p(src_row), rows, hidden, p(out), stream()), "desta_embed_gather")


def gather_rows(src, idx, rows, hidden, out):
    check(_gather(p(src), p(idx), rows, hidden, p(out), stream()), "desta_gather_rows_bf16")


@_profiled("causal_lm_loss", lambda logits, ld, labels, batch, seq, vocab, loss, write_grad=True: (2 + 2 * int(write_grad)) * batch * (seq - 1) * vocab)
def causal_lm_loss(logits, ld, labels, batch, seq, vocab, loss, write_grad=True):
    ws = scratch(lib.desta_ce_workspace_floats(batch, seq), logits.device, "ce")
    check(_ce(p(logits), ld, p(labels), batch, seq, vocab, p(loss), p(ws), int(write_grad), stream()),
          "desta_causal_lm_loss")


@_profiled("token_logprobs", lambda logits, ld, labels, rows, vocab, out, is_top1=None: 2 * rows * vocab)
def token_logprobs(logits, ld, labels, rows, vocab, out, is_top1=None):
    check(_token_logprobs(p(logits), ld, p(labels), rows, vocab, p(out), p(is_top1), stream()), "desta_token_logprobs")


@_profiled("topk_logprobs", lambda logits, ld, tokens, rows, vocab, top_n, token_logprob=None, top_ids=None, top_logprobs=None: 4 * rows * vocab)
def topk_logprobs(logits, ld, tokens, rows, vocab, top_n, token_logprob=None, top_ids=None, top_logprobs=None):
    global TOPK_LOGPROBS_CALLS
    check(_topk_logprobs(p(logits), ld, p(tokens), rows, vocab, top_n, p(token_logprob), p(top_ids), p(top_logprobs), stream()),
          "desta_topk_logprobs")
    TOPK_LOGPROBS_CALLS += 1


def tap_mix_fwd(x, lw, taps, batch, prompt, d, out):
    check(_mix_fwd(p(x), p(lw), taps, batch, prompt, d, p(out), stream()), "desta_tap_mix_fwd")


def tap_mix_bwd(x, lw, dout, taps, batch, prompt, d, dx, dlw):
    check(_mix_bwd(p(x), p(lw), p(dout), taps, batch, prompt, d, p(dx), p(dlw), stream()), "desta_tap_mix_bwd")


class AttnDesc(C.Structure):
    _fields_ = [("Q", vp), ("K", vp), ("V", vp), ("O", vp), ("dO", vp), ("dQ", vp), ("dK", vp), ("dV", vp),
                ("lse", vp),
                ("q_batch_stride", i64), ("q_row_stride", i64), ("k_batch_stride", i64), ("k_row_stride", i64),
                ("v_batch_stride", i64), ("v_row_stride", i64), ("o_batch_stride", i64), ("o_row_stride", i64),
                ("do_batch_stride", i64), ("do_row_stride", i64), ("dq_batch_stride", i64), ("dq_row_stride", i64),
                ("dk_batch_stride", i64), ("dk_row_stride", i64), ("dv_batch_stride", i64), ("dv_row_stride", i64),
                ("batch", i32), ("n_q_heads", i32), ("n_kv_heads", i32), ("seq_q", i32), ("seq_k", i32),
                ("head_dim", i32), ("causal", i32), ("kv_start", vp), ("scale", f32),
                ("dropout_p", f32), ("dropout_seed", C.c_uint64), ("rope_cos_sin", vp), ("O_f32", vp),
                ("dkv_transposed", i32), ("dkv_t_ld", i64), ("dkv_bias_grad", vp)]


_attn_fwd = _sig("desta_attention_fwd", C.POINTER(AttnDesc), vp)
lib.desta_attention_bwd_workspace_floats.restype = c_size_t
lib.desta_attention_bwd_workspace_floats.argtypes = [i32, i32, i32]
_attn_bwd = _sig("desta_attention_bwd", C.POINTER(AttnDesc), vp, vp)


def _elem_ptr(t, offset_elems):
    return t.data_ptr() + offset_elems * t.element_size()


def attn_desc(q, k, v, o, lse, *, batch, hq, hkv, sq, sk, hd, scale, causal=False, kv_start=None,
              q_off=0, k_off=0, v_off=0, q_rs=None, k_rs=None, v_rs=None, o_rs=None, dropout_p=0.0, dropout_seed=0,
              q_bs=None, k_bs=None, v_bs=None, o_bs=None, o_f32=None):
    d = AttnDesc()
    q_rs = q.shape[-1] if q_rs is None else q_rs
    k_rs = k.shape[-1] if k_rs is None else k_rs
    v_rs = v.shape[-1] if v_rs is None else v_rs
    o_rs = o.shape[-1] if o_rs is None else o_rs
    d.Q, d.K, d.V, d.O = _elem_ptr(q, q_off), _elem_ptr(k, k_off), _elem_ptr(v, v_off), p(o)
    d.lse = p(lse)
    d.q_row_stride, d.q_batch_stride = q_rs, (sq * q_rs if q_bs is None else q_bs)
    d.k_row_stride, d.k_batch_stride = k_rs, (sk * k_rs if k_bs is None else k_bs)
    d.v_row_stride, d.v_batch_stride = v_rs, (sk * v_rs if v_bs is None else v_bs)
    d.o_row_stride, d.o_batch_stride = o_rs, (sq * o_rs if o_bs is None else o_bs)
    d.batch, d.n_q_heads, d.n_kv_heads, d.seq_q, d.seq_k, d.head_dim = batch, hq, hkv, sq, sk, hd
    d.causal = int(causal)
    d.kv_start = p(kv_start)
    d.scale = scale
    d.dropout_p, d.dropout_seed = dropout_p, dropout_seed
    if o_f32 is not None:
        assert o_f32.dtype == torch.float32 and o_f32.shape == o.shape and o_f32.is_contiguous() and o.is_contiguous()
    d.O_f32 = p(o_f32)
    d._keep = (q, k, v, o, lse, kv_start, o_f32)
    return d


def _attn_flops(d, mult):
    f = 4.0 * d.batch * d.n_q_heads * d.seq_q * d.seq_k * d.head_dim
    return mult * (f * 0.5 if d.causal else f)


def _attn_tag(d, *a, **k):
    return f"D{d.head_dim}{'c' if d.causal else ''}_q{d.seq_q}_k{d.seq_k}"


@_profiled(lambda d: "attn_fwd:" + _attn_tag(d), lambda d: _attn_flops(d, 1.0))
def attention_fwd(d: AttnDesc):
    check(_attn_fwd(C.byref(d), stream()), "desta_attention_fwd")


lib.desta_attention_decode_chunk.restype = i32
lib.desta_attention_decode_workspace_bytes.restype = c_size_t
lib.desta_attention_decode_workspace_bytes.argtypes = [i32, i32, i32, i32]
_attn_decode = _sig("desta_attention_decode", C.POINTER(AttnDesc), vp, c_size_t, vp)
DECODE_ATTN_CHUNK = int(lib.desta_attention_decode_chunk())
DECODE_ATTN_MIN_KEYS = 448
ATTN_DECODE_CALLS = 0


def attention_decode_workspace_bytes(batch: int, hq: int, sk: int, hd: int = 128) -> int:
    return int(lib.desta_attention_decode_workspace_bytes(int(batch), int(hq), int(sk), int(hd)))


@_profiled(lambda d, *a, **k: "attn_decode:" + _attn_tag(d), lambda d, *a, **k: _attn_flops(d, 1.0))
def attention_decode(d: AttnDesc, ws=None):
    global ATTN_DECODE_CALLS
    check(_attn_decode(C.byref(d), p(ws), 0 if ws is None else ws.numel() * ws.element_size(), stream()), "desta_attention_decode")
    ATTN_DECODE_CALLS += 1


_attn_kv8 = _sig("desta_attention_decode_kv8", C.POINTER(AttnDesc), vp, vp, i64, i64, vp, c_size_t, vp)
ATTN_KV8_CALLS = 0


@_profiled(lambda d, *a, **k: "attn_kv8:" + _attn_tag(d), lambda d, *a, **k: _attn_flops(d, 1.0))
def attention_decode_kv8(d: AttnDesc, k_scale, v_scale, scale_bs, scale_rs, ws=None):
    global ATTN_KV8_CALLS
    check(_attn_kv8(C.byref(d), p(k_scale), p(v_scale), int(scale_bs), int(scale_rs), p(ws),
                    0 if ws is None else ws.numel() * ws.element_size(), stream()), "desta_attention_decode_kv8")
    ATTN_KV8_CALLS += 1


_kv8_dequant = _sig("desta_kv8_dequant", vp, i64, i64, vp, i64, i64, vp, i32, i32, i32, i32, vp, i64, i64, vp)
KV8_DEQUANT_CALLS = 0


@_profiled("kv8_dequant", lambda *a, **k: 3.0 * a[7] * a[10] * a[8] * a[9])
def kv8_dequant(cache, kv_bs, kv_rs, scale, scale_bs, scale_rs, kv_start, batch, n_heads, hd, slot1, out, out_bs, out_rs):
    global KV8_DEQUANT_CALLS
    check(_kv8_dequant(p(cache), int(kv_bs), int(kv_rs), p(scale), int(scale_bs), int(scale_rs), p(kv_start), int(batch), int(n_heads),
                       int(hd), int(slot1), p(out), int(out_bs), int(out_rs), stream()), "desta_kv8_dequant")
    KV8_DEQUANT_CALLS += 1


@_profiled(lambda d, *a, **k: "attn_bwd:" + _attn_tag(d), lambda d, *a, **k: _attn_flops(d, 2.5))
def attention_bwd(d: AttnDesc, do, dq, dk=None, dv=None, *, do_rs=None, dq_off=0, dk_off=0, dv_off=0, dq_rs=None,
                  dk_rs=None, dv_rs=None, do_bs=None, dq_bs=None, dk_bs=None, dv_bs=None, rope_cos_sin=None, dkv_t=None):
    d.rope_cos_sin = p(rope_cos_sin)
    d._keep_rope = rope_cos_sin
    do_rs = do.shape[-1] if do_rs is None else do_rs
    dq_rs = dq.shape[-1] if dq_rs is None else dq_rs
    d.dO, d.do_row_stride, d.do_batch_stride = p(do), do_rs, (d.seq_q * do_rs if do_bs is None else do_bs)
    d.dQ, d.dq_row_stride, d.dq_batch_stride = _elem_ptr(dq, dq_off), dq_rs, (d.seq_q * dq_rs if dq_bs is None else dq_bs)
    d.dkv_transposed, d.dkv_t_ld, d.dkv_bias_grad = 0, 0, 0
    if dkv_t is not None:
        t, ld, bias = dkv_t
        assert dk is None and dv is None and t.dtype == torch.bfloat16 and (bias is None or bias.dtype == torch.float32)
        d.dK, d.dV = p(t), _elem_ptr(t, d.n_q_heads * d.head_dim * ld)
        d.dkv_transposed, d.dkv_t_ld, d.dkv_bias_grad = 1, ld, p(bias)
        dk = dv = t
    elif dk is not None:
        dk_rs = dk.shape[-1] if dk_rs is None else dk_rs
        dv_rs = dv.shape[-1] if dv_rs is None else dv_rs
        d.dK, d.dk_row_stride, d.dk_batch_stride = _elem_ptr(dk, dk_off), dk_rs, (d.seq_k * dk_rs if dk_bs is None else dk_bs)
        d.dV, d.dv_row_stride, d.dv_batch_stride = _elem_ptr(dv, dv_off), dv_rs, (d.seq_k * dv_rs if dv_bs is None else dv_bs)
    else:
        d.dK = d.dV = 0
    ws = scratch(lib.desta_attention_bwd_workspace_floats(d.batch, d.n_q_heads, d.seq_q), do.device, "attn")
    d._keep_bwd = (do, dq, dk, dv, ws)
    check(_attn_bwd(C.byref(d), p(ws), stream()), "desta_attention_bwd")


_prompt_expand = _sig("desta_prompt_expand", vp, i32, i32, i64, vp, vp, vp)
_prompt_grad = _sig("desta_prompt_grad", vp, i32, i32, i64, vp, vp)


def prompt_expand(prompts, taps, batch, n, x32, x16):
    check(_prompt_expand(p(prompts), taps, batch, n, p(x32), p(x16), stream()), "desta_prompt_expand")


def prompt_grad(dx, taps, batch, n, dprompts):
    check(_prompt_grad(p(dx), taps, batch, n, p(dprompts), stream()), "desta_prompt_grad")


def gemm_force_variant(v: int) -> None:
    lib.desta_gemm_force_variant.argtypes = [i32]
    lib.desta_gemm_force_variant(v)


_dropout = _sig("desta_dropout_bf16", vp, vp, i32, i32, i64, f32, C.c_uint64, vp)
_dropout_mask = _sig("desta_dropout_mask_u8", C.c_uint64, i64, f32, vp, vp)


def dropout_bf16(x, y, rows, cols, ld, p_drop, seed):
    check(_dropout(p(x), p(y), rows, cols, ld, p_drop, seed, stream()), "desta_dropout_bf16")


def dropout_mask(seed, n, p_drop, device="cuda"):
    out = torch.empty(n, dtype=torch.uint8, device=device)
    check(_dropout_mask(seed, n, p_drop, p(out), stream()), "desta_dropout_mask_u8")
    return out


def gemm_set_persistent(on: bool) -> None:
    lib.desta_gemm_set_persistent.argtypes = [i32]
    lib.desta_gemm_set_persistent(int(on))


def gemm_set_option(option: int, value: int) -> None:
    lib.desta_gemm_set_option.argtypes = [i32, i32]
    check(lib.desta_gemm_set_option(option, value), "desta_gemm_set_option")


_argmax = _sig("desta_argmax_bf16", vp, i64, i32, i32, vp, vp, vp)
lib.desta_argmax_workspace_bytes.restype = C.c_size_t
lib.desta_argmax_workspace_bytes.argtypes = [i32]
_argmax_ws = {}


def argmax_bf16(x, ld, rows, cols, out):
    key = (x.device, rows)
    ws = _argmax_ws.get(key)
    if ws is None:
        ws = _argmax_ws[key] = torch.empty(lib.desta_argmax_workspace_bytes(rows), dtype=torch.uint8, device=x.device)
    check(_argmax(p(x), ld, rows, cols, p(out), p(ws), stream()), "desta_argmax_bf16")


_mask_tokens = _sig("desta_mask_tokens_bf16", vp, i64, i32, i32, vp, i32, vp)


def mask_tokens_bf16(logits, ld, rows, cols, ids):
    check(_mask_tokens(p(logits), ld, rows, cols, p(ids), int(ids.numel()), stream()), "desta_mask_tokens_bf16")


_rope_kv = _sig("desta_rope_kv_append", vp, i64, i32, i32, i32, i32, i32, vp, vp, vp, f32, vp, vp, i64, i64, i32, vp)


def rope_kv_append(buf, ld, rows, seq, n_q, n_kv, hd, cos_sin, q_norm_w, k_norm_w, eps, pos_shift, cache, kv_bs, kv_rs, slot0):
    check(_rope_kv(p(buf), ld, rows, seq, n_q, n_kv, hd, p(cos_sin), p(q_norm_w), p(k_norm_w), eps, p(pos_shift), p(cache), kv_bs,
                   kv_rs, slot0, stream()), "desta_rope_kv_append")


_rope_kv8 = _sig("desta_rope_kv_append_e4m3", vp, i64, i32, i32, i32, i32, i32, vp, vp, vp, f32, vp, vp, i64, i64, vp, i64, i64, i32, vp)


def rope_kv_append_e4m3(buf, ld, rows, seq, n_q, n_kv, hd, cos_sin, q_norm_w, k_norm_w, eps, pos_shift, cache, kv_bs, kv_rs,
                        scale, scale_bs, scale_rs, slot0):
    check(_rope_kv8(p(buf), ld, rows, seq, n_q, n_kv, hd, p(cos_sin), p(q_norm_w), p(k_norm_w), eps, p(pos_shift), p(cache), kv_bs,
                    kv_rs, p(scale), scale_bs, scale_rs, slot0, stream()), "desta_rope_kv_append_e4m3")


_sample = _sig("desta_sample_top_p_bf16", vp, i64, i32, i32, f32, f32, C.c_uint64, C.c_uint32, vp, vp, vp)


def sample_top_p(logits, ld, rows, cols, temperature, top_p, seed, step, out, keep_mask=None):
    check(_sample(p(logits), ld, rows, cols, temperature, top_p, seed & 0xFFFFFFFFFFFFFFFF, step & 0xFFFFFFFF, p(out), p(keep_mask),
                  stream()), "desta_sample_top_p_bf16")


_sample_chain = _sig("desta_sample_bf16", vp, i64, i32, i32, vp, i64, i32, f32, i32, f32, i32, f32, f32, C.c_uint64, C.c_uint32,
                     vp, vp, vp)


def sample(logits, ld, rows, cols, out, *, do_sample=True, temperature=1.0, top_k=0, top_p=1.0, min_p=0.0, repetition_penalty=1.0,
           hist=None, hist_len=0, seed=0, step=0, keep_mask=None):
    hist_ld = 0 if hist is None else hist.stride(0)
    check(_sample_chain(p(logits), ld, rows, cols, p(hist), hist_ld, hist_len, repetition_penalty, int(bool(do_sample)), temperature,
                        top_k, top_p, min_p, seed & 0xFFFFFFFFFFFFFFFF, step & 0xFFFFFFFF, p(out), p(keep_mask), stream()),
          "desta_sample_bf16")


class CommUniqueId(C.Structure):
    _fields_ = [("internal", C.c_char * 128)]


def comm_get_unique_id() -> bytes:
    lib.desta_comm_get_unique_id.argtypes = [C.POINTER(CommUniqueId)]
    uid = CommUniqueId()
    check(lib.desta_comm_get_unique_id(C.byref(uid)), "desta_comm_get_unique_id")
    return bytes(C.string_at(C.addressof(uid), 128))


def comm_create(world_size: int, rank: int, unique_id: bytes) -> int:
    lib.desta_comm_create.argtypes = [C.POINTER(vp), i32, i32, C.POINTER(CommUniqueId)]
    uid = CommUniqueId()
    C.memmove(C.addressof(uid), unique_id, 128)
    comm = vp()
    check(lib.desta_comm_create(C.byref(comm), world_size, rank, C.byref(uid)), "desta_comm_create")
    return comm.value


def allreduce_grads(comm: int, grads: torch.Tensor) -> None:
    assert grads.dtype == torch.float32 and grads.is_contiguous()
    lib.desta_allreduce_grads.argtypes = [vp, vp, i64, vp]
    check(lib.desta_allreduce_grads(comm, p(grads), grads.numel(), stream()), "desta_allreduce_grads")


def comm_destroy(comm: int) -> None:
    lib.desta_comm_destroy.argtypes = [vp]
    check(lib.desta_comm_destroy(comm), "desta_comm_destroy")


class Context:

    def __init__(self, device: int = 0):
        lib.desta_create.argtypes = [i32, C.POINTER(vp)]
        h = vp()
        check(lib.desta_create(int(device), C.byref(h)), "desta_create")
        self.handle = h.value

    def info(self) -> dict:
        lib.desta_handle_info.argtypes = [vp, C.POINTER(i32), C.POINTER(i32), C.c_char_p, C.c_size_t]
        dev, cus, arch = i32(), i32(), C.create_string_buffer(64)
        check(lib.desta_handle_info(self.handle, C.byref(dev), C.byref(cus), arch, 64), "desta_handle_info")
        return {"device": dev.value, "compute_units": cus.value, "arch": arch.value.decode()}

    def last_error(self) -> str:
        lib.desta_handle_last_error.argtypes = [vp]
        lib.desta_handle_last_error.restype = C.c_char_p
        return lib.desta_handle_last_error(self.handle).decode()

    def close(self) -> None:
        if self.handle:
# ... 119 lines not shown
```

desta2.5-audio_amd/desta/models/modeling_desta25.py:

```python
from __future__ import annotations

import json
import logging
import math
import os
from collections import OrderedDict
from dataclasses import dataclass, field, asdict
from typing import Dict, List, Optional, Sequence, Tuple

import torch

from .. import _hip as H
from ..optim import ParamArena

BF16, F32 = torch.bfloat16, torch.float32
ENC = "perception.whisper.model.encoder."
CON = "perception.connector."
LLM = "llm_model."

TAP_LAYERS = {
    "whisper-tiny": [0, 1, 2, 3], "whisper-small": [2, 5, 8, 11], "whisper-medium": [5, 11, 17, 23],
    "whisper-large-v3": [7, 15, 23, 31], "whisper-large-v3-turbo": [7, 15, 23, 31],
}
_TAPS_BY_DEPTH = {4: [0, 1, 2, 3], 12: [2, 5, 8, 11], 24: [5, 11, 17, 23], 32: [7, 15, 23, 31]}
# ... 1707 lines not shown
                             q_rs=self.qkvw, k_rs=self.kvw, v_rs=self.kvw, o_rs=self.hq * self.hd,
                             q_bs=self.qkvw, k_bs=Smax * self.kvw, v_bs=Smax * self.kvw, o_bs=self.hq * self.hd)
            if kv8:
                H.attention_decode_kv8(ad, sc, self.kv_scale_v[li], Smax * 2 * self.hkv, 2 * self.hkv, self.g_attn_ws)
            elif split_kv:
                H.attention_decode(ad, self.g_attn_ws)
            else:
                H.attention_fwd(ad)
            mm(self.g_att, ly["wo"], q8.get("wo"), self.g_xm, h, self.hq * self.hd, residual=x)
            proj(self.g_xm, ly["n2"], ly["wgu"], q8.get("wgu"), self.g_act, self.I, act=4)
            mm(self.g_act, ly["wd"], q8.get("wd"), self.g_x, h, self.I, residual=self.g_xm)
            if layer_hook is not None:
                layer_hook(li, self.g_x)
        proj(self.g_x, self.norm, self.head, self.head8 if fp8 else None, self.g_logits, self.V, ldc=self.Vp)
        return self.g_logits

    def generate_greedy(self, x0_filler, B: int, S: int, kv_start: torch.Tensor, max_new_tokens: int, pad_token_id: int,
                        eos_token_ids=None, forced_tokens: Optional[torch.Tensor] = None, collect_logits: bool = False,
                        do_sample: bool = False, temperature: float = 1.0, top_p: float = 1.0, seed: int = 0, layer_hook=None,
                        after_prompt=None, top_k: Optional[int] = None, min_p: Optional[float] = None,
                        repetition_penalty: Optional[float] = None, prompt_ids: Optional[torch.Tensor] = None, chunk_hook=None,
                        logprobs: Optional[int] = None):
        assert max_new_tokens >= 1
        check_decode_rows(B)
        use_pen = repetition_penalty is not None and float(repetition_penalty) != 1.0
        chain = use_pen or (do_sample and ((top_k is not None and int(top_k) != 0) or (min_p is not None and float(min_p) > 0.0)))
        Smax = S + max_new_tokens
        self._gen_alloc(B, Smax)
        dev = self.dev
        kv_start = kv_start.to(torch.int32).contiguous()
        neg_pad = (-kv_start).contiguous()
        if self.prefill_chunk is not None:
            logits = self.prefill(x0_filler, B, S, kv_start, self.g_logits, layer_hook=layer_hook, chunk_hook=chunk_hook)
        else:
            logits = self.forward(x0_filler, B, S, kv_start, None, False, pos_shift=neg_pad, cos_sin=self.gen_cos_sin, last_logits=self.g_logits,
                                  kv_cache=self.kv_cache, layer_hook=layer_hook)
        if after_prompt is not None:
            after_prompt()
        out = torch.full((B, max_new_tokens), int(pad_token_id), dtype=torch.int64, device=dev)
        P = 0
        if chain:
            P = 0 if prompt_ids is None else int(prompt_ids.shape[1])
            hist = torch.full((B, P + max_new_tokens), int(pad_token_id), dtype=torch.int64, device=dev)
            if P:
                hist[:, :P] = prompt_ids.to(dev, torch.int64)
            out = hist[:, P:]
        steps_logits = []
        if logprobs is not None:
            lp_tok = torch.zeros(B, max_new_tokens, dtype=F32, device=dev)
            lp_ids = torch.full((B, max_new_tokens, logprobs), -1, dtype=torch.int32, device=dev)
            lp_top = torch.zeros(B, max_new_tokens, logprobs, dtype=F32, device=dev)
            st_tok = torch.empty(B, dtype=F32, device=dev)
            st_ids = torch.empty(B, logprobs, dtype=torch.int32, device=dev)
            st_top = torch.empty(B, logprobs, dtype=F32, device=dev)
        finished = torch.zeros(B, dtype=torch.bool, device=dev)
        eos = None if not eos_token_ids else torch.tensor(list(eos_token_ids), dtype=torch.int64, device=dev)
        n_new = 0
        for t in range(max_new_tokens):
            if collect_logits:
                steps_logits.append(logits[:, :self.V].clone())
            if chain:
                H.sample(logits, self.Vp, B, self.V, self.g_next, do_sample=do_sample, temperature=float(temperature),
                         top_k=int(top_k or 0), top_p=float(top_p), min_p=float(min_p or 0.0),
                         repetition_penalty=float(repetition_penalty) if use_pen else 1.0, hist=hist, hist_len=P + t, seed=seed, step=t)
            elif do_sample:
                H.sample_top_p(logits, self.Vp, B, self.V, float(temperature), float(top_p), seed, t, self.g_next)
            else:
                H.argmax_bf16(logits, self.Vp, B, self.V, self.g_next)
            nxt = self.g_next if forced_tokens is None else forced_tokens[:, t].to(dev, torch.int64)
            nxt = torch.where(finished, torch.full_like(nxt, int(pad_token_id)), nxt)
            out[:, t] = nxt
            if logprobs is not None:
                H.topk_logprobs(logits, self.Vp, torch.where(finished, torch.full_like(nxt, -1), nxt), B, self.V, logprobs, st_tok, st_ids, st_top)
                lp_tok[:, t] = st_tok
                lp_ids[:, t] = st_ids
                lp_top[:, t] = st_top
            n_new = t + 1
            if eos is not None:
                finished |= (nxt.unsqueeze(1) == eos.unsqueeze(0)).any(dim=1)
                if (t & 7) == 7 and bool(finished.all()):
                    break
            if t + 1 == max_new_tokens:
                break
            cur = S + t
            shift = (cur - kv_start).to(torch.int32).contiguous()
            logits = self.decode_step(nxt, cur, kv_start, shift, layer_hook=layer_hook)
        if eos is not None and n_new > 1:
            done_at = (out.unsqueeze(2) == eos.view(1, 1, -1)).any(dim=2).int().argmax(dim=1)
            has = (out.unsqueeze(2) == eos.view(1, 1, -1)).any(dim=2).any(dim=1)
            last = int(torch.where(has, done_at + 1, torch.full_like(done_at, n_new)).max())
            n_new = min(n_new, last)
        out = out[:, :n_new]
        res = (out, torch.stack(steps_logits[:n_new])) if collect_logits else (out,)
        if logprobs is not None:
            res += (TokenLogprobs(token_logprobs=lp_tok[:, :n_new], top_ids=lp_ids[:, :n_new], top_logprobs=lp_top[:, :n_new]),)
        return res if len(res) > 1 else out

    def loss_and_grad(self, labels: torch.Tensor, write_grad: bool) -> torch.Tensor:
        if getattr(self, "compact", None) is not None:
            idx, lab_c, Mc = self.compact
            if Mc == 0:
                self.loss.zero_()
                return self.loss
            H.causal_lm_loss(self.logits, self.Vp, lab_c, 1, Mc + 1, self.V, self.loss, write_grad=write_grad)
            return self.loss
        H.causal_lm_loss(self.logits, self.Vp, labels, self.B, self.S, self.V, self.loss, write_grad=write_grad)
        return self.loss

    def backward(self, first_needed_pos: int = 0, out_rows: Optional[Tuple[int, int]] = None, layer_hook_bwd=None) -> torch.Tensor:
        c, h, M, S, B = self.c, self.h, self.M, self.S, self.B
        if self.lora is not None:
            first_needed_pos, out_rows = 0, None
        r0 = first_needed_pos * B if self.s_major else 0
        Mr = M - r0
        tl = max(self.tail0, r0) if self.s_major else r0
        smb = B if self.s_major else 0
        dhb = self.hb
        if getattr(self, "compact", None) is not None and self.compact[2] == 0:
            self.dxa.zero_()
            return self.dxa
        if getattr(self, "compact", None) is not None:
            idx, _, Mc = self.compact
            H.gemm(self.logits, self.headT, self.hbc, Mc, h, self.Vp, ldb=self.Vp)
            dhb[r0:].zero_()
            H.scatter_rows(self.hbc, idx, Mc, h, dhb)
        else:
            H.gemm(self.logits, self.headT, dhb, M, h, self.Vp, ldb=self.Vp)
        dx, other = self.dxa, self.dxb
        if tl > r0:
            dx[r0:tl].zero_()
            other[r0:tl].zero_()
            self.datt[r0:tl].zero_()
        if M - tl > 0:
            H.rmsnorm_bwd(dhb[tl:], self.xs[self.L][tl:], self.norm, self.rf[tl:], dx[tl:])
        aw = self.hq * self.hd
        for i in reversed(range(self.L)):
            ly, s = self.layers[i], self.sv[i]
            if layer_hook_bwd is not None:
                layer_hook_bwd(i, dx)
            a0 = tl if i == self.L - 1 else r0
            Ma = M - a0
            if Ma > 0:
                if s.get("gu_blocked"):
                    H.gemm(dx[a0:], ly["wdT"], self.dgu[a0:], Ma, self.I, h, act=3, aux=s["gu"][a0:], ld_aux=2 * self.I, ldc=2 * self.I)
                    H.gemm(self.dgu[a0:], ly["wguT_b"], dhb[a0:], Ma, h, 2 * self.I)
                else:
                    if "wguT" not in ly:
                        ly["wguT"] = self._T(ly["wgu"])
                    H.gemm(dx[a0:], ly["wdT"], self.act[a0:], Ma, self.I, h)
                    H.swiglu_bwd(s["gu"][a0:], self.act[a0:], self.dgu[a0:], Ma, self.I)
                    H.gemm(self.dgu[a0:], ly["wguT"], dhb[a0:], Ma, h, 2 * self.I)
                H.rmsnorm_bwd(dhb[a0:], s["xm"][a0:], ly["n2"], s["r2"][a0:], other[a0:], dres=dx[a0:])
                H.gemm(other[a0:], ly["woT"], self.datt[a0:], Ma, aw, h)
            fused = getattr(self, "_rope_fused", False)
            rcs = self.cos_sin_il if fused else None
            if self.s_major:
                H.attention_bwd(s["ad"], self.datt, self.dqkv, self.dqkv, self.dqkv, dq_off=0, dk_off=aw, dv_off=(self.hq + self.hkv) * self.hd,
                                do_rs=B * aw, dq_rs=B * self.qkvw, dk_rs=B * self.qkvw, dv_rs=B * self.qkvw,
                                do_bs=aw, dq_bs=self.qkvw, dk_bs=self.qkvw, dv_bs=self.qkvw, rope_cos_sin=rcs)
            else:
                H.attention_bwd(s["ad"], self.datt, self.dqkv, self.dqkv, self.dqkv, dq_off=0, dk_off=aw, dv_off=(self.hq + self.hkv) * self.hd,
                                rope_cos_sin=rcs)
            if not fused:
                H.rope(self.dqkv, self.qkvw, M, S, self.hq, self.hkv, self.hd, self.cos_sin, ly.get("qn"), ly.get("kn"), c.rms_norm_eps,
                       pre_norm=s.get("pre"), ld_pre=self.qkvw, backward=True, s_major_batch=smb)
            o0, o1 = r0, M
            if i == 0 and out_rows is not None and self.s_major and self.skip_dead_rows:
                o0, o1 = max(r0, out_rows[0] * B), min(M, out_rows[1] * B)
            H.gemm(self.dqkv[o0:], ly["wqkvT_il" if fused else "wqkvT"], dhb[o0:], o1 - o0, h, self.qkvw)
            if self.lora is not None:
                self._lora_bwd(i, ly, s, dhb, M)
            H.rmsnorm_bwd(dhb[o0:o1], self.xs[i][o0:o1], ly["n1"], s["r1"][o0:o1], dx[o0:o1], dres=other[o0:o1])
        return dx


class DeSTA25AudioModel:
    config_class = DeSTA25Config

    def __init__(self, config: DeSTA25Config, weights: Optional[Dict[str, torch.Tensor]] = None, device="cuda:0", **kwargs):
        if not torch.cuda.is_available():
            raise RuntimeError("DeSTA25AudioModel (MI355X hot path) needs a HIP device; there is no CPU fallback")
        self.config = config
        self.device = torch.device(device)
        self.audio_locator, self.placeholder_token = config.audio_locator, config.placeholder_token
        if weights is None:
            weights = self._load_base_weights(config)
        shapes = connector_param_shapes(config)
        shapes.update(lora_param_shapes(config))
        self.arena = ParamArena(list(shapes.items()), self.device)
        self.trainable_parameter_names = list(shapes.keys())
        with torch.cuda.device(self.device):
            self.encoder = WhisperEncoderHIP(config, weights, self.device)
            self.llm = CausalLMHIP(config, weights, self.device)
            self.connector = QformerConnectorHIP(config, self.arena, self.device)
            if config.use_lora:
                self.llm.attach_lora(self.arena, config.lora_r, config.lora_alpha, config.lora_dropout)
            self.orca = OrcaHIP(config, self.connector, self.device) if config.connector_mode == "orca_hybrid" else None
            gp = os.path.join(str(config.llm_model_id), "generation_config.json")
            self.llm_generation_config = {}
            if os.path.isfile(gp):
                with open(gp) as f:
                    self.llm_generation_config = json.load(f)
            self.asr_decoder = None
            if (DEC + "embed_tokens.weight") in weights:
                gc = config.extra.get("whisper_generation_config")
                if gc is None:
                    gp = os.path.join(config.encoder_model_id, "generation_config.json")
                    if os.path.isfile(gp):
                        with open(gp) as f:
                            gc = json.load(f)
                self.asr_decoder = WhisperDecoderHIP(config, weights, self.device, gc)
        self.audio_tokens = config.orca_global_num_tokens if self.orca is not None else config.prompt_size
        self._init_connector(weights)
        e = config.encoder_config
        self.enc_all = None
        self._enc_bufs: List[Optional[torch.Tensor]] = [None, None]
        self._enc_cur = 0
        self.training = True
        self._weights_dirty = True
        self._fwd = None
        self._enc_pending: List[tuple] = []
        self.dropout_seed = 0
        self.compact_lm_head = True
        self._tr_stream = self._tr_idx = self._tr_lab = self._tr_count = self._tr_count_host = None
        self._fwd_count = 0
        self._slot_cache: Dict[tuple, tuple] = {}

    @staticmethod
    def _load_base_weights(config) -> Dict[str, torch.Tensor]:
        from safetensors import safe_open
        out: Dict[str, torch.Tensor] = {}
        for path, prefix, keep in ((config.llm_model_id, LLM, None), (config.encoder_model_id, "perception.whisper.", ("model.encoder.", "model.decoder."))):
            files = sorted(f for f in os.listdir(path) if f.endswith(".safetensors")) if os.path.isdir(path) else []
            if not files:
                raise FileNotFoundError(f"no *.safetensors under '{path}' (local HF model directory required; no hub access)")
            for fn in files:
                with safe_open(os.path.join(path, fn), framework="pt") as f:
                    for k in f.keys():
                        if keep is None or k.startswith(keep):
                            out[prefix + k] = f.get_tensor(k)
        return out

    def _init_connector(self, weights):
        g = torch.Generator().manual_seed(0)
        for name, shape in self.arena.shapes.items():
            if name in weights:
                self.arena.param(name).copy_(weights[name].to(self.device, F32).reshape(shape))
                continue
            if ".lora_B." in name:
                v = torch.zeros(*shape)
            elif "layer_prompts" in name or "global_queries" in name:
                v = torch.randn(*shape, generator=g)
            elif name.endswith("layer_weights"):
                v = torch.zeros(*shape)
            elif "LayerNorm" in name or "proj.0." in name.replace("gate_proj", "") or ".local_ln." in name or ".ln." in name:
                v = torch.ones(*shape) if name.endswith("weight") else torch.zeros(*shape)
            elif name.endswith("gate_proj.2.weight"):
                v = torch.zeros(*shape)
            elif name.endswith("gate_proj.2.bias"):
                v = torch.full(shape, self.config.orca_gate_init)
            elif name.endswith("in_proj_weight"):
                v = (torch.rand(*shape, generator=g) * 2 - 1) * math.sqrt(6.0 / (shape[0] + shape[1]))
            elif name.endswith("in_proj_bias") or name.endswith("cross_attn.out_proj.bias"):
                v = torch.zeros(*shape)
            elif name.endswith(".weight"):
                v = (torch.rand(*shape, generator=g) * 2 - 1) / math.sqrt(int(math.prod(shape[1:])))
            else:
                fan_in = int(math.prod(self.arena.shapes[name[:-4] + "weight"][1:]))
                v = (torch.rand(*shape, generator=g) * 2 - 1) / math.sqrt(fan_in)
            self.arena.param(name).copy_(v.to(self.device))

    def named_parameters(self):
        for n in self.trainable_parameter_names:
            yield n, self.arena.param(n)

    def state_dict(self):
        return OrderedDict((n, self.arena.param(n).detach().clone()) for n in sorted(self.trainable_parameter_names))

    def load_state_dict(self, state_dict, strict=True, assign=False):
        sd = {k.replace("ocar_cross_attns", "orca_cross_attns"): v for k, v in state_dict.items()}
        glw = sd.get(CON + "global_layer_weights")
        if glw is not None and self.orca is not None and int(glw.shape[1]) != len(self.config.target_layer_ids):
            self.config.align_orca_layers(int(glw.shape[1]))
            logging.warning("checkpoint taps %d encoder layers: rebuilding the ORCA connector (orca_use_all_layers=%s)", glw.shape[1], self.config.orca_use_all_layers)
            shapes = connector_param_shapes(self.config)
            shapes.update(lora_param_shapes(self.config))
            self.arena = ParamArena(list(shapes.items()), self.device)
            self.trainable_parameter_names = list(shapes.keys())
            with torch.cuda.device(self.device):
                self.connector = QformerConnectorHIP(self.config, self.arena, self.device)
                if self.config.use_lora:
                    self.llm.attach_lora(self.arena, self.config.lora_r, self.config.lora_alpha, self.config.lora_dropout)
                self.orca = OrcaHIP(self.config, self.connector, self.device)
            self._init_connector({})
            self.drop_prefetched()
            self.encoder.B = 0
            self.enc_all, self._enc_bufs = None, [None, None]
        missing = [n for n in self.trainable_parameter_names if n not in sd]
        unexpected = [k for k in sd if k not in self.arena.shapes]
        if strict and (missing or unexpected):
            raise RuntimeError(f"Error(s) in loading state_dict: missing {missing[:5]} unexpected {unexpected[:5]}")
        for n in self.trainable_parameter_names:
            if n in sd:
                self.arena.param(n).copy_(sd[n].to(self.device, F32).reshape(self.arena.shapes[n]))
        self._weights_dirty = True
        return missing, unexpected

    def save_pretrained(self, path: str, state_dict=None, **kwargs):
        from safetensors.torch import save_file
        os.makedirs(path, exist_ok=True)
        self.config.save_pretrained(path)
        sd = state_dict if state_dict is not None else self.state_dict()
# ... 589 lines not shown
```

include/desta_hip.h:

```cpp
#ifndef DESTA_HIP_H
#define DESTA_HIP_H

#include <stddef.h>
#include <stdint.h>

#ifdef __cplusplus
extern "C" {
#endif

#define DESTA_ABI_VERSION 8

int desta_abi_version(void);
size_t desta_sizeof_desc(int which);
const char* desta_last_error(void);

typedef struct desta_context* desta_handle;
int desta_create(int device, desta_handle* out);
int desta_destroy(desta_handle h);
int desta_handle_info(desta_handle h, int* device, int* compute_units, char* arch, size_t arch_bytes);
const char* desta_handle_last_error(desta_handle h);

typedef struct desta_gemm_desc {
    const void* A; const void* B; void* C;
    int M, N, K, batch;
// ... 7 lines not shown
    int out_f32;
    void* preact;
    int64_t ldp, stride_p;
    float alpha;
    void* aux;
    int64_t ld_aux;
    float dropout_p;
    uint64_t dropout_seed;
    void* workspace;
    size_t workspace_bytes;
    int trans_a, trans_b;
    const float* a_rms_weight;
    float a_rms_eps;
    const float* rope_cos_sin;
    const int32_t* rope_pos;
    int rope_cols, rope_head_dim;
} desta_gemm_desc;
int desta_gemm_bf16_nt(const desta_gemm_desc* d, void* stream);
int desta_gemm_force_variant(int variant);
int desta_gemm_last_kernel(void);
int desta_gemm_set_persistent(int on);
int desta_gemm_set_option(int option, int value);

int desta_quantize_rows_e4m3(const void* w_bf16, int rows, int cols, int64_t ld, uint8_t* q, float* scale, void* stream);
int desta_gemm_w8a16_nt(const desta_gemm_desc* d, const float* b_scale, void* stream);

int desta_gemm_wide_nt(const desta_gemm_desc* d, const float* b_scale, void* stream);

typedef struct desta_opt_plan {
    const int64_t* tensors; const float* tensor_wd; int n_tensors;
    const int32_t* units; const int64_t* unit_col_off; int n_units;
    const int64_t* vecs; const float* vec_wd; int n_vec;
    int64_t state_floats;
    int max_cols;
    const int32_t* chunks; const int32_t* ten_chunks; int n_chunks;
    const int32_t* fin; int n_fin;
    int64_t colpart_floats;
    const int32_t* group_bounds; int n_groups;
    const int32_t* ragged_units; int n_ragged;
} desta_opt_plan;
size_t desta_adafactor_workspace_floats(const desta_opt_plan* plan);
int desta_clip_adafactor_step(const desta_opt_plan* plan, float* params, const float* grads, float* state,
                              float* workspace, float lr, float beta2t, float eps1, float clip_threshold,
                              float max_grad_norm, void* stream);

#define DESTA_ADAMW_ITEM_FLOATS 4096
typedef struct desta_adamw_plan {
    const int64_t* items; const float* item_wd; int n_items;
    int64_t numel;
} desta_adamw_plan;
size_t desta_adamw_workspace_floats(const desta_adamw_plan* plan);
int desta_clip_adamw_step(const desta_adamw_plan* plan, float* params, const float* grads, float* exp_avg, float* exp_avg_sq,
                          float* workspace, float lr, double beta1, double beta2, float eps, float bc1, float bc2,
                          float max_grad_norm, void* stream);

size_t desta_logmel_table_floats(int n_mels);
size_t desta_logmel_workspace_floats(int batch);
int desta_logmel_fill_tables(int n_mels, float* host_out);
int desta_logmel_f32(const float* wave, int batch, int n_samples, int64_t wave_stride, const float* tables,
                     int n_mels, float* out, float* workspace, void* stream);

int desta_layernorm_fwd(const void* x, int x_f32, const float* gamma, const float* beta, float eps, int rows,
                        int cols, void* y_bf16, float* y_f32, float* stats, void* stream);
size_t desta_layernorm_bwd_workspace_floats(int rows, int cols);
int desta_layernorm_bwd(const void* dy, int dy_f32, const void* x, int x_f32, const float* gamma,
                        const float* stats, int rows, int cols, float* dx_f32, void* dx_bf16, float* dgamma,
                        float* dbeta, int accumulate, float* workspace, void* stream);
int desta_rmsnorm_fwd(const void* x, const float* weight, float eps, int rows, int cols, void* y, float* rstd,
                      void* stream);
int desta_rmsnorm_bwd(const void* dy, const void* x, const float* weight, const float* rstd, const void* dres,
                      int rows, int cols, void* dx, void* stream);

size_t desta_colsum_workspace_floats(int rows, int cols);
int desta_colsum_bf16(const void* x, int rows, int cols, int64_t ld, float* out, int accumulate,
                      float* workspace, void* stream);

int desta_rope(void* buf, int64_t ld, int rows, int seq, int n_q_heads, int n_kv_heads, int head_dim,
               const float* cos_sin, const float* q_norm_w, const float* k_norm_w, float eps,
               const void* pre_norm, int64_t ld_pre, int backward, const int32_t* pos_shift, int s_major_batch, void* stream);

int desta_swiglu_fwd(const void* gate_up, void* act, int64_t rows, int inter, void* stream);
int desta_swiglu_bwd(const void* gate_up, const void* dact, void* dgate_up, int64_t rows, int inter, void* stream);
int desta_gelu_bwd(const void* preact, const void* dact, void* dpre, int64_t n, void* stream);
int desta_cast_f32_bf16(const float* x, void* y, int64_t n, void* stream);
int desta_add_f32(float* y, const float* x, int64_t n, void* stream);
int desta_transpose_to_bf16(const void* in, int in_f32, int64_t ld_in, int rows, int cols, void* out,
                            int64_t ld_out, void* stream);
int desta_mel_to_rows(const float* mel, int batch, int n_mels, int frames, int c_pad, void* out, void* stream);

int desta_embed_gather(const void* table, const void* audio_rows, const int32_t* src_row, int rows, int hidden,
                       void* out, void* stream);
int desta_gather_rows_bf16(const void* in, const int32_t* idx, int rows, int hidden, void* out, void* stream);

size_t desta_ce_workspace_floats(int batch, int seq);
int desta_causal_lm_loss(void* logits, int64_t ld, const int64_t* labels, int batch, int seq, int vocab,
                         float* loss, float* workspace, int write_grad, void* stream);

int desta_token_logprobs(const void* logits_bf16, int64_t ld, const int64_t* labels, int rows, int vocab,
                         float* logprob, uint8_t* is_top1 , void* stream);

int desta_topk_logprobs(const void* logits_bf16, int64_t ld, const int64_t* tokens , int rows, int vocab,
                        int top_n, float* token_logprob ,
                        int32_t* top_ids , float* top_logprobs , void* stream);

int desta_tap_mix_fwd(const float* x, const float* layer_weights, int taps, int batch, int prompt, int d,
                      float* out, void* stream);
int desta_tap_mix_bwd(const float* x, const float* layer_weights, const float* dout, int taps, int batch,
                      int prompt, int d, float* dx, float* dlayer_weights, void* stream);

int desta_orca_local_mix(const void* x, const float* layer_weights, int taps, int64_t rows, int d, void* out, void* stream);
int desta_orca_rope(const void* x, void* y, int batch, int tokens, int hidden, float theta, float position_scale, int round_cos_sin, void* stream);
int desta_orca_gate_residual(void* hidden, int64_t ld_hidden, const void* cross, const void* gate_hidden, const float* gate_w2, const float* gate_b2,
                             int64_t rows, int hidden_size, int gate_width, float* gate_out, void* stream);
int desta_orca_sim_loss(const void* x, const void* y, const int32_t* y_index, int batch, int nx, int ny, int64_t y_rows, int hidden,
                        int subtract_identity, float* partials, void* stream);
int desta_orca_align(const void* audio, int tokens, const void* hidden, int64_t hidden_row_stride, int64_t hidden_batch_stride, int hidden_size,
                     const int32_t* spans, int n_spans, float* out, void* stream);
int desta_orca_gate_residual_bwd(const void* d_out, int64_t ld, const void* cross, const float* gate, int64_t rows, int hidden_size, void* d_cross,
                                 float* d_gate_pre, void* stream);
int desta_orca_gate_mlp_bwd(const float* d_gate_pre, const void* gate_preact, const void* gate_hidden, const float* gate_w2, int64_t rows, int gate_width,
                            void* d_preact, float* d_w2, float* d_b2, float* workspace, void* stream);
int desta_orca_align_bwd(const void* audio, int tokens, const void* hidden, int64_t hidden_row_stride, int64_t hidden_batch_stride, int hidden_size,
                         const int32_t* spans, int n_spans, float coef, void* d_hidden, int64_t d_row_stride, int64_t d_batch_stride, void* stream);
int desta_orca_rope_bwd(const float* d_rotated, int batch, int tokens, int hidden, float theta, float position_scale, int round_cos_sin, int n_first,
                        float* d_first, float* d_rest, void* stream);
int desta_orca_col2im_add(const void* d_col, int batch, int tokens_out, int tokens_padded, int hidden, int kernel, int stride, void* d_padded, void* stream);
int desta_orca_local_mix_bwd(const void* d_out, const void* x, const float* layer_weights, int taps, int64_t rows, int d, float* d_layer_weights,
                             float* workspace, void* stream);
int desta_orca_sim_loss_bwd(const void* x, const int32_t* x_index, int64_t x_rows, const void* y, const int32_t* y_index, int64_t y_rows, int batch, int nx,
                            int ny, int hidden, int subtract_identity, float coef, float* d_x, void* stream);

typedef struct desta_attn_desc {
    const void* Q; const void* K; const void* V; void* O;
    const void* dO; void* dQ; void* dK; void* dV;
    float* lse;
    int64_t q_batch_stride, q_row_stride, k_batch_stride, k_row_stride, v_batch_stride, v_row_stride;
    int64_t o_batch_stride, o_row_stride, do_batch_stride, do_row_stride;
    int64_t dq_batch_stride, dq_row_stride, dk_batch_stride, dk_row_stride, dv_batch_stride, dv_row_stride;
    int batch, n_q_heads, n_kv_heads, seq_q, seq_k, head_dim;
    int causal;
    const int32_t* kv_start;
    float scale;
    float dropout_p;
    uint64_t dropout_seed;
    const float* rope_cos_sin;
    float* O_f32;
    int dkv_transposed;
    int64_t dkv_t_ld;
    float* dkv_bias_grad;
} desta_attn_desc;
int desta_attention_fwd(const desta_attn_desc* d, void* stream);
size_t desta_attention_bwd_workspace_floats(int batch, int n_q_heads, int seq_q);
int desta_attention_bwd(const desta_attn_desc* d, float* workspace, void* stream);
int desta_attention_set_concurrent_bwd(int on);
int desta_attention_set_option(int which, int value);

#ifndef DESTA_ATTN_DECODE_CHUNK
#define DESTA_ATTN_DECODE_CHUNK 256
#endif
int    desta_attention_decode_chunk(void);
size_t desta_attention_decode_workspace_bytes(int batch, int n_q_heads, int seq_k, int head_dim);
int    desta_attention_decode(const desta_attn_desc* d, void* workspace, size_t workspace_bytes, void* stream);

int    desta_attention_decode_kv8(const desta_attn_desc* d, const float* k_scale, const float* v_scale, int64_t scale_batch_stride,
                                  int64_t scale_row_stride, void* workspace, size_t workspace_bytes, void* stream);

int    desta_kv8_dequant(const uint8_t* kv_cache, int64_t kv_batch_stride, int64_t kv_row_stride, const float* kv_scale,
                         int64_t scale_batch_stride, int64_t scale_row_stride, const int32_t* kv_start, int batch, int n_heads,
                         int head_dim, int slot1, void* out_bf16, int64_t out_batch_stride, int64_t out_row_stride, void* stream);

int desta_prompt_expand(const float* prompts, int taps, int batch, int64_t n, float* x_f32, void* x_bf16, void* stream);
int desta_prompt_grad(const float* dx, int taps, int batch, int64_t n, float* dprompts, void* stream);

int desta_dropout_bf16(const void* x, void* y, int rows, int cols, int64_t ld, float p, uint64_t seed, void* stream);
int desta_dropout_mask_u8(uint64_t seed, int64_t n, float p, uint8_t* out, void* stream);

int desta_target_rows(const int64_t* labels, int batch, int seq, int32_t* idx, int64_t* compact_labels, int32_t* count,
                      int s_major, void* stream);
int desta_scatter_rows_bf16(const void* in, const int32_t* idx, int rows, int hidden, void* out, void* stream);

size_t desta_argmax_workspace_bytes(int rows);
int desta_mask_tokens_bf16(void* logits, int64_t ld, int rows, int cols, const int32_t* ids, int n, void* stream);
int desta_argmax_bf16(const void* x, int64_t ld, int rows, int cols, int64_t* out, void* workspace, void* stream);

int desta_sample_top_p_bf16(const void* logits, int64_t ld, int rows, int cols, float temperature, float top_p,
                            uint64_t seed, uint32_t step, int64_t* out, uint8_t* keep_mask, void* stream);

int desta_sample_bf16(const void* logits, int64_t ld, int rows, int cols, const int64_t* hist, int64_t hist_ld, int hist_len,
                      float repetition_penalty, int do_sample, float temperature, int top_k, float top_p, float min_p,
                      uint64_t seed, uint32_t step, int64_t* out, uint8_t* keep_mask, void* stream);

int desta_rope_kv_append(void* qkv, int64_t ld, int rows, int seq, int n_q_heads, int n_kv_heads, int head_dim,
                         const float* cos_sin, const float* q_norm_w, const float* k_norm_w, float eps,
                         const int32_t* pos_shift, void* kv_cache, int64_t kv_batch_stride, int64_t kv_row_stride,
                         int slot0, void* stream);

int desta_rope_kv_append_e4m3(void* qkv, int64_t ld, int rows, int seq, int n_q_heads, int n_kv_heads, int head_dim,
                              const float* cos_sin, const float* q_norm_w, const float* k_norm_w, float eps,
                              const int32_t* pos_shift, uint8_t* kv_cache, int64_t kv_batch_stride, int64_t kv_row_stride,
                              float* kv_scale, int64_t scale_batch_stride, int64_t scale_row_stride, int slot0, void* stream);

typedef struct { char internal[128]; } desta_comm_unique_id;
typedef void* desta_comm;
int desta_comm_get_unique_id(desta_comm_unique_id* id);
int desta_comm_create(desta_comm* comm, int world_size, int rank, const desta_comm_unique_id* id);
int desta_allreduce_grads(desta_comm comm, float* grads, int64_t n, void* stream);
int desta_comm_destroy(desta_comm comm);

#ifdef __cplusplus
}
#endif
#endif
```

Measured before the change: 6.547.

## Skip dead-row attention gradients and split dK/dV waves into producer roles

Adds a grad_from bound to attention backward so dQ and dK/dV kernels skip query and key blocks whose gradients are not needed (rows before the first live row in the first layer). It also adds a role-split dK/dV kernel variant, on by default through option 6. That variant runs eight waves: half compute dK while the other half load Q/dO into double-buffered LDS and compute dV, so loads overlap compute and each wave needs fewer accumulator registers. The cost is more LDS, a larger block, and recomputing S in both roles.

After: 6.578, median of 6. No clear change (+0.5%).

```diff
diff --git a/desta2.5-audio_amd/csrc/attention.hip b/desta2.5-audio_amd/csrc/attention.hip
--- a/desta2.5-audio_amd/csrc/attention.hip
+++ b/desta2.5-audio_amd/csrc/attention.hip
@@ -25,6 +25,7 @@
     float scale;
     unsigned drop_thresh, seed_lo, seed_hi; float drop_scale;
     long dkv_t_ld;
+    int grad_from;
 };
 
 template <int D>
@@ -40,12 +41,12 @@
 template <int D, int ROWS, int NT = 256> using stage_t = typename stage_vec<ROWS * (D / 8) / NT>::type;
 
 template <int D, int ROWS, int NT = 256>
-__device__ __forceinline__ stage_t<D, ROWS, NT> tile_load(const bf16_t* base, long rs, int row0, int max_row) {
+__device__ __forceinline__ stage_t<D, ROWS, NT> tile_load(const bf16_t* base, long rs, int row0, int max_row, int tid) {
     constexpr int CH = D / 8, N = ROWS * CH / NT;
     stage_t<D, ROWS, NT> out;
 #pragma unroll
     for (int i = 0; i < N; ++i) {
-        const int id = i * NT + threadIdx.x;
+        const int id = i * NT + tid;
         const int r = id / CH, c = id % CH;
         const int gr = min(row0 + r, max_row);
         const uint4 v = *(const uint4*)(base + (long)gr * rs + c * 8);
@@ -54,15 +55,21 @@
     return out;
 }
 template <int D, int ROWS, int NT = 256>
-__device__ __forceinline__ void tile_store(char* img, const stage_t<D, ROWS, NT>& regs) {
+__device__ __forceinline__ stage_t<D, ROWS, NT> tile_load(const bf16_t* base, long rs, int row0, int max_row) {
+    return tile_load<D, ROWS, NT>(base, rs, row0, max_row, (int)threadIdx.x);
+}
+template <int D, int ROWS, int NT = 256>
+__device__ __forceinline__ void tile_store(char* img, const stage_t<D, ROWS, NT>& regs, int tid) {
     constexpr int CH = D / 8, N = ROWS * CH / NT;
 #pragma unroll
     for (int i = 0; i < N; ++i) {
-        const int id = i * NT + threadIdx.x;
+        const int id = i * NT + tid;
         const int r = id / CH, c = id % CH;
         *(uint4*)(img + img_off<D>(r, c)) = make_uint4(regs[4 * i + 0], regs[4 * i + 1], regs[4 * i + 2], regs[4 * i + 3]);
     }
 }
+template <int D, int ROWS, int NT = 256>
+__device__ __forceinline__ void tile_store(char* img, const stage_t<D, ROWS, NT>& regs) { tile_store<D, ROWS, NT>(img, regs, (int)threadIdx.x); }
 
 template <int D>
 __device__ __forceinline__ bf16x8 frag_rows(const char* img, int row0, int ks, int lane) {
@@ -795,8 +802,9 @@
     const int b = g / p.Hkv, hk = g % p.Hkv;
     const int h = hk * G + hg * HPB + wave / WPH;
     const int qb0 = qblk * RB, q0 = qb0 + (wave % WPH) * 32;
+    if (qb0 + RB <= p.grad_from) return;
     const int qcol = q0 + (lane & 31), qc = min(qcol, p.Sq - 1);
-    const bool wave_on = q0 < p.Sq;
+    const bool wave_on = q0 < p.Sq && q0 + 32 > p.grad_from;
 
     const int coff = p.Sk - p.Sq;
     const int kv_lo = p.kv_start ? max(0, min(p.kv_start[b], p.Sk)) : 0;
@@ -986,11 +994,14 @@
 #define ATTN_DKDV_QR 32
 #endif
 
-template <int D, bool DROP, int NW = 4>
+template <int D, bool DROP, int NW = 4, bool SPLIT = false>
 __global__ __launch_bounds__(64 * NW, (NW == 4 && D == 64) ? 2 : 1) void attn_bwd_dkdv_k(AttnArgs p) {
+    static_assert(!SPLIT || (NW == 8 && D == 128 && !DROP), "the role split is built for eight waves, D = 128, no dropout");
     constexpr int QR = (D == 128) ? ATTN_DKDV_QR : 32;
-    constexpr int NT = 64 * NW, KB = 32 * NW;
-    constexpr int LDS_LOOP = 2 * QR * D * 2 + 2 * QR * 4, LDS_EPI = NW * 32 * 64 * 4;
+    constexpr int KW = SPLIT ? NW / 2 : NW;
+    constexpr int NT = 64 * NW, KB = 32 * KW;
+    constexpr int LDS_BUF = 2 * QR * D * 2 + 2 * QR * 4;
+    constexpr int LDS_LOOP = (SPLIT ? 2 : 1) * LDS_BUF, LDS_EPI = NW * 32 * 64 * 4;
     __shared__ __attribute__((aligned(16))) char lds[LDS_LOOP > LDS_EPI ? LDS_LOOP : LDS_EPI];
     char* qimg = lds;
     char* gimg = lds + QR * D * 2;
@@ -998,7 +1009,10 @@
     float* dlt_s = lse_s + QR;
     const int lane = threadIdx.x & 63, wave = __builtin_amdgcn_readfirstlane(threadIdx.x >> 6), h2 = lane >> 5;
     const int nhb = p.Hkv * p.B;
-    const int kb0 = (blockIdx.x / nhb) * KB, k0 = kb0 + wave * 32;
+    const int kb0 = (blockIdx.x / nhb) * KB, k0 = kb0 + (SPLIT ? wave % KW : wave) * 32;
+    if (kb0 + KB <= p.grad_from) return;
+    const bool dv_role = SPLIT && wave >= KW;
+    const bool dead = k0 + 32 <= p.grad_from;
     const int hk = (blockIdx.x % nhb) % p.Hkv, b = (blockIdx.x % nhb) / p.Hkv, group = p.Hq / p.Hkv;
     const int kcol = k0 + (lane & 31), kc = min(kcol, p.Sk - 1);
     const int kv_lo = p.kv_start ? max(0, min(p.kv_start[b], p.Sk)) : 0;
@@ -1006,32 +1020,35 @@
 
     const bf16_t* kptr = p.K + (long)b * p.k_bs + (long)kc * p.k_rs + (long)hk * D;
     const bf16_t* vptr = p.V + (long)b * p.v_bs + (long)kc * p.v_rs + (long)hk * D;
-    bf16x8 kf[D / 16], vf[D / 16];
-#pragma unroll
-    for (int ds = 0; ds < D / 16; ++ds) {
-        kf[ds] = *(const bf16x8*)(kptr + 16 * ds + 8 * h2);
-        vf[ds] = *(const bf16x8*)(vptr + 16 * ds + 8 * h2);
+    bf16x8 kf[D / 16], vf[D / 16] = {};
+#pragma unroll
+    for (int ds = 0; ds < D / 16; ++ds) kf[ds] = *(const bf16x8*)(kptr + 16 * ds + 8 * h2);
+    if (!dv_role) {
+#pragma unroll
+        for (int ds = 0; ds < D / 16; ++ds) vf[ds] = *(const bf16x8*)(vptr + 16 * ds + 8 * h2);
     }
     const bool key_ok = kcol < p.Sk && kcol >= kv_lo;
 
-    f32x16 dk[D / 32], dv[D / 32];
+    f32x16 dk[D / 32], dv[SPLIT ? 1 : D / 32];
 #pragma unroll
     for (int i = 0; i < D / 32; ++i)
 #pragma unroll
-        for (int r = 0; r < 16; ++r) { dk[i][r] = 0.f; dv[i][r] = 0.f; }
-
-    const int q_first = p.causal ? max(0, kb0 - coff) : 0;
+        for (int r = 0; r < 16; ++r) { dk[i][r] = 0.f; if constexpr (!SPLIT) dv[i][r] = 0.f; }
+
+    const int q_first = max(p.causal ? max(0, kb0 - coff) : 0, p.grad_from);
     const int qt_lo = q_first / QR, qt_hi = (p.Sq + QR - 1) / QR;
     const int nq = qt_hi - qt_lo, n_it = group * nq;
-    stage_t<D, QR, NT> qr0 = {}, gr0 = {}, qr1 = {}, gr1 = {};
+    constexpr int ST = SPLIT ? 64 * KW : NT;
+    const int stid = (int)threadIdx.x - (NT - ST);
+    stage_t<D, QR, ST> qr0 = {}, gr0 = {}, qr1 = {}, gr1 = {};
     float ls0 = 0.f, dl0 = 0.f, ls1 = 0.f, dl1 = 0.f;
 #define DESTA_Q_FETCH(IT, QR_, GR, LS, DL)                                                                      \
     {                                                                                                          \
         const int h_ = hk * group + (IT) / nq, qt_ = qt_lo + (IT) % nq;                                        \
-        QR_ = tile_load<D, QR, NT>(p.Q + (long)b * p.q_bs + (long)h_ * D, p.q_rs, qt_ * QR, p.Sq - 1);        \
-        GR = tile_load<D, QR, NT>(p.dO + (long)b * p.do_bs + (long)h_ * D, p.do_rs, qt_ * QR, p.Sq - 1);      \
-        if (threadIdx.x < QR) {                                                                                \
-            const long st_ = ((long)b * p.Hq + h_) * p.Sq + min(qt_ * QR + (int)threadIdx.x, p.Sq - 1);       \
+        QR_ = tile_load<D, QR, ST>(p.Q + (long)b * p.q_bs + (long)h_ * D, p.q_rs, qt_ * QR, p.Sq - 1, stid);  \
+        GR = tile_load<D, QR, ST>(p.dO + (long)b * p.do_bs + (long)h_ * D, p.do_rs, qt_ * QR, p.Sq - 1, stid);\
+        if (stid < QR) {                                                                                       \
+            const long st_ = ((long)b * p.Hq + h_) * p.Sq + min(qt_ * QR + stid, p.Sq - 1);                   \
             LS = p.lse[st_];                                                                                   \
             DL = p.delta[st_];                                                                                 \
         }                                                                                                      \
@@ -1039,14 +1056,21 @@
 #define DESTA_Q_STAGE(IT, QR_, GR, LS, DL)                                                                      \
     __syncthreads();                                                                                           \
     asm volatile("; stage " #QR_ ::: "memory");                                                                \
-    tile_store<D, QR, NT>(qimg, QR_);                                                                          \
-    tile_store<D, QR, NT>(gimg, GR);                                                                           \
-    if (threadIdx.x < QR) { lse_s[threadIdx.x] = LS; dlt_s[threadIdx.x] = DL; }                                \
+    tile_store<D, QR, ST>(qimg, QR_, stid);                                                                    \
+    tile_store<D, QR, ST>(gimg, GR, stid);                                                                     \
+    if (stid < QR) { lse_s[stid] = LS; dlt_s[stid] = DL; }                                                     \
     __syncthreads();                                                                                           \
     if ((IT) + 2 < n_it) DESTA_Q_FETCH((IT) + 2, QR_, GR, LS, DL)
-    if (n_it > 0) DESTA_Q_FETCH(0, qr0, gr0, ls0, dl0)
-    if (n_it > 1) DESTA_Q_FETCH(1, qr1, gr1, ls1, dl1)
-    auto compute = [&](const int it) __attribute__((always_inline)) {
+#define DESTA_Q_PUT(BO, NEXT, QR_, GR, LS, DL)                                                                  \
+    tile_store<D, QR, ST>(qimg + (BO), QR_, stid);                                                             \
+    tile_store<D, QR, ST>(gimg + (BO), GR, stid);                                                              \
+    if (stid < QR) { ((float*)((char*)lse_s + (BO)))[stid] = LS; ((float*)((char*)dlt_s + (BO)))[stid] = DL; } \
+    if ((NEXT) < n_it) DESTA_Q_FETCH(NEXT, QR_, GR, LS, DL)
+    auto compute = [&](const int it, const int bo, const bool dvr) __attribute__((always_inline)) {
+        const char* qimg = lds + bo;
+        const char* gimg = lds + bo + QR * D * 2;
+        const float* lse_s = (const float*)(lds + bo + 2 * QR * D * 2);
+        const float* dlt_s = lse_s + QR;
         const int qt = qt_lo + it % nq;
         constexpr int NS = QR / 32;
         f32x16 stv[NS], dpv[NS];
@@ -1054,10 +1078,16 @@
 #pragma unroll
         for (int sub = 0; sub < NS; ++sub) {
             const int qb = qt * QR + sub * 32;
-            act[sub] = qb < p.Sq && !(p.causal && k0 > qb + 31 + coff);
+            act[sub] = qb < p.Sq && qb + 32 > p.grad_from && !dead && !(p.causal && k0 > qb + 31 + coff);
             if (!act[sub]) continue;
 #pragma unroll
             for (int r = 0; r < 16; ++r) { stv[sub][r] = 0.f; dpv[sub][r] = 0.f; }
+            if (dvr) {
+#pragma unroll
+                for (int ds = 0; ds < D / 16; ++ds)
+                    stv[sub] = __builtin_amdgcn_mfma_f32_32x32x16_bf16(frag_rows<D>(qimg, sub * 32, ds, lane), kf[ds], stv[sub], 0, 0, 0);
+                continue;
+            }
 #pragma unroll
             for (int ds = 0; ds < D / 16; ++ds) {
                 stv[sub] = __builtin_amdgcn_mfma_f32_32x32x16_bf16(frag_rows<D>(qimg, sub * 32, ds, lane), kf[ds], stv[sub], 0, 0, 0);
@@ -1076,9 +1106,14 @@
 #pragma unroll
             for (int q4 = 0; q4 < 4; ++q4) {
                 const float4 a4 = *(const float4*)(lse_s + sub * 32 + 8 * q4 + 4 * h2);
-                const float4 b4 = *(const float4*)(dlt_s + sub * 32 + 8 * q4 + 4 * h2);
                 lsv[4 * q4 + 0] = a4.x; lsv[4 * q4 + 1] = a4.y; lsv[4 * q4 + 2] = a4.z; lsv[4 * q4 + 3] = a4.w;
-                dlv[4 * q4 + 0] = b4.x; dlv[4 * q4 + 1] = b4.y; dlv[4 * q4 + 2] = b4.z; dlv[4 * q4 + 3] = b4.w;
+            }
+            if (!dvr) {
+#pragma unroll
+                for (int q4 = 0; q4 < 4; ++q4) {
+                    const float4 b4 = *(const float4*)(dlt_s + sub * 32 + 8 * q4 + 4 * h2);
+                    dlv[4 * q4 + 0] = b4.x; dlv[4 * q4 + 1] = b4.y; dlv[4 * q4 + 2] = b4.z; dlv[4 * q4 + 3] = b4.w;
+                }
             }
             unsigned keep = 0xffffu;
             if constexpr (DROP) {
@@ -1108,6 +1143,18 @@
                     st[r] = ok ? st[r] : -INFINITY;
                 }
             }
+            if (dvr) {
+#pragma unroll
+                for (int r = 0; r < 16; ++r) st[r] = __builtin_amdgcn_exp2f(fmaf(st[r], p.scale_log2, -lsv[r]));
+#pragma unroll
+                for (int s = 0; s < 2; ++s) {
+                    const bf16x8 pf = acc_frag(st, s);
+#pragma unroll
+                    for (int i = 0; i < D / 32; ++i)
+                        dk[i] = __builtin_amdgcn_mfma_f32_32x32x16_bf16(pf, frag_tr<D>(gimg, sub * 32 + 16 * s, i * 32, lane), dk[i], 0, 0, 0);
+                }
+                continue;
+            }
 #pragma unroll
             for (int r = 0; r < 16; ++r) {
                 const float pv = __builtin_amdgcn_exp2f(fmaf(st[r], p.scale_log2, -lsv[r]));
@@ -1121,20 +1168,52 @@
                 const bf16x8 pf = acc_frag(st, s), dsf = acc_frag(dp, s);
 #pragma unroll
                 for (int i = 0; i < D / 32; ++i) {
-                    dv[i] = __builtin_amdgcn_mfma_f32_32x32x16_bf16(pf, frag_tr<D>(gimg, sub * 32 + 16 * s, i * 32, lane), dv[i], 0, 0, 0);
+                    if constexpr (!SPLIT) dv[i] = __builtin_amdgcn_mfma_f32_32x32x16_bf16(pf, frag_tr<D>(gimg, sub * 32 + 16 * s, i * 32, lane), dv[i], 0, 0, 0);
                     dk[i] = __builtin_amdgcn_mfma_f32_32x32x16_bf16(dsf, frag_tr<D>(qimg, sub * 32 + 16 * s, i * 32, lane), dk[i], 0, 0, 0);
                 }
             }
         }
     };
-    for (int it = 0; it < n_it; it += 2) {
-        DESTA_Q_STAGE(it, qr0, gr0, ls0, dl0)
-        compute(it);
-        if (it + 1 < n_it) {
-            DESTA_Q_STAGE(it + 1, qr1, gr1, ls1, dl1)
-            compute(it + 1);
-        }
-    }
+    if constexpr (SPLIT) {
+        if (dv_role) {
+            if (n_it > 0) DESTA_Q_FETCH(0, qr0, gr0, ls0, dl0)
+            if (n_it > 1) DESTA_Q_FETCH(1, qr1, gr1, ls1, dl1)
+            if (n_it > 0) { DESTA_Q_PUT(0, 2, qr0, gr0, ls0, dl0) }
+            __syncthreads();
+            for (int it = 0; it < n_it; it += 2) {
+                if (it + 1 < n_it) { DESTA_Q_PUT(LDS_BUF, it + 3, qr1, gr1, ls1, dl1) }
+                compute(it, 0, true);
+                __syncthreads();
+                if (it + 1 < n_it) {
+                    if (it + 2 < n_it) { DESTA_Q_PUT(0, it + 4, qr0, gr0, ls0, dl0) }
+                    compute(it + 1, LDS_BUF, true);
+                    __syncthreads();
+                }
+            }
+        } else {
+            __syncthreads();
+            for (int it = 0; it < n_it; it += 2) {
+                compute(it, 0, false);
+                __syncthreads();
+                if (it + 1 < n_it) {
+                    compute(it + 1, LDS_BUF, false);
+                    __syncthreads();
+                }
+            }
+        }
+    } else {
+        if (n_it > 0) DESTA_Q_FETCH(0, qr0, gr0, ls0, dl0)
+        if (n_it > 1) DESTA_Q_FETCH(1, qr1, gr1, ls1, dl1)
+        for (int it = 0; it < n_it; it += 2) {
+            DESTA_Q_STAGE(it, qr0, gr0, ls0, dl0)
+            compute(it, 0, false);
+            if (it + 1 < n_it) {
+                DESTA_Q_STAGE(it + 1, qr1, gr1, ls1, dl1)
+                compute(it + 1, 0, false);
+            }
+        }
+    }
+#undef DESTA_Q_PUT
 #undef DESTA_Q_STAGE
 #undef DESTA_Q_FETCH
     bf16_t* dkp = p.dK + (long)b * p.dk_bs + (long)hk * D;
@@ -1170,18 +1249,30 @@
                 asm volatile("s_waitcnt lgkmcnt(0)" ::: "memory");
             }
         };
-        emit(dk, dkp, p.dk_rs, p.rope_cs != nullptr);
-        emit(dv, dvp, p.dv_rs, false);
+        if (dead) return;
+        if constexpr (SPLIT) {
+            if (dv_role) emit(dk, dvp, p.dv_rs, false);
+            else emit(dk, dkp, p.dk_rs, p.rope_cs != nullptr);
+        } else {
+            emit(dk, dkp, p.dk_rs, p.rope_cs != nullptr);
+            emit(dv, dvp, p.dv_rs, false);
+        }
         return;
     }
+    if (dead) return;
 #pragma unroll
     for (int i = 0; i < D / 32; ++i)
 #pragma unroll
         for (int r = 0; r < 16; ++r) {
             const int key = k0 + acc_row(r, lane);
             if (key < p.Sk) {
-                dkp[(long)key * p.dk_rs + i * 32 + (lane & 31)] = f2bf(dk[i][r]);
-                dvp[(long)key * p.dv_rs + i * 32 + (lane & 31)] = f2bf(dv[i][r]);
+                if constexpr (SPLIT) {
+                    if (dv_role) dvp[(long)key * p.dv_rs + i * 32 + (lane & 31)] = f2bf(dk[i][r]);
+                    else dkp[(long)key * p.dk_rs + i * 32 + (lane & 31)] = f2bf(dk[i][r]);
+                } else {
+                    dkp[(long)key * p.dk_rs + i * 32 + (lane & 31)] = f2bf(dk[i][r]);
+                    dvp[(long)key * p.dv_rs + i * 32 + (lane & 31)] = f2bf(dv[i][r]);
+                }
             }
         }
 }
@@ -1887,12 +1978,13 @@
     a.drop_scale = 1.0f / (1.0f - d->dropout_p);
     a.seed_lo = (unsigned)d->dropout_seed; a.seed_hi = (unsigned)(d->dropout_seed >> 32);
     a.dkv_t_ld = d->dkv_transposed ? d->dkv_t_ld : 0;
+    a.grad_from = 0;
     return DESTA_OK;
 }
 
 }
 
-namespace { int g_attn_opt[8] = {1, 0, 0, 0, 1, 0, 0, 0}; }
+namespace { int g_attn_opt[8] = {1, 0, 0, 0, 1, 0, 1, 0}; }
 extern "C" int desta_attention_set_option(int which, int value) {
     DESTA_CHECK_ARG(which >= 0 && which < 8, "attention_set_option: unknown option %d", which);
     g_attn_opt[which] = value;
@@ -2142,9 +2234,22 @@
     return DESTA_OK;
 }
 
+namespace {
+void launch_dkdv128(const AttnArgs& a, dim3 grid, hipStream_t st) {
+    if (g_attn_opt[6]) hipLaunchKernelGGL((attn_bwd_dkdv_k<128, false, 8, true>), grid, dim3(512), 0, st, a);
+    else hipLaunchKernelGGL((attn_bwd_dkdv_k<128, false>), grid, dim3(256), 0, st, a);
+}
+}
+
 extern "C" int desta_attention_bwd(const desta_attn_desc* d, float* workspace, void* stream) {
+    return desta_attention_bwd_from(d, 0, workspace, stream);
+}
+
+extern "C" int desta_attention_bwd_from(const desta_attn_desc* d, int grad_from, float* workspace, void* stream) {
     AttnArgs a;
     if (int rc = fill_args(d, a)) return rc;
+    DESTA_CHECK_ARG(grad_from <= 0 || d->seq_q == d->seq_k, "attention_bwd_from: grad_from needs seq_q == seq_k");
+    a.grad_from = grad_from < 0 ? 0 : (grad_from > a.Sq ? a.Sq : grad_from);
     DESTA_CHECK_ARG(d->O && d->dO && d->lse && workspace && d->dQ, "attention_bwd: null argument");
     DESTA_CHECK_ARG((d->dK == nullptr) == (d->dV == nullptr), "attention_bwd: dK and dV go together");
     DESTA_CHECK_ARG(d->dq_row_stride % 4 == 0 && d->do_row_stride % 8 == 0 && d->o_row_stride % 8 == 0,
@@ -2176,7 +2281,7 @@
                 if (g_attn_opt[5] && a.causal) {
                     dim3 gk2((unsigned)((a.Sk + 63) / 64) * a.Hkv * a.B);
                     hipLaunchKernelGGL((attn_bwd_dkdv_k<128, false, 2>), gk2, dim3(128), 0, st, a);
-                } else hipLaunchKernelGGL((attn_bwd_dkdv_k<128, false>), gk_, dim3(256), 0, st, a);
+                } else launch_dkdv128(a, gk_, st);
             }
         } else {
             if (!a.causal) hipLaunchKernelGGL((attn_bwd_dq8_k<64, false, 1>), g8, dim3(512), 0, st, a, workspace);
@@ -2219,13 +2324,13 @@
         hipLaunchKernelGGL(attn_delta_k<128>, gd, dim3(256), 0, st, a, workspace);
         BwdFork* f = (g_bwd_concurrent && d->dK) ? bwd_fork() : nullptr;
         if (f && hipEventRecord(f->fork, st) == hipSuccess && hipStreamWaitEvent(f->side, f->fork, 0) == hipSuccess) {
-            hipLaunchKernelGGL((attn_bwd_dkdv_k<128, false>), gk, dim3(256), 0, st, a);
+            launch_dkdv128(a, gk, st);
             hipLaunchKernelGGL((attn_bwd_dq_k<128, false>), gq, dim3(256), 0, f->side, a);
             DESTA_CHECK_ARG(hipEventRecord(f->join, f->side) == hipSuccess && hipStreamWaitEvent(st, f->join, 0) == hipSuccess,
                             "attention_bwd: could not join the side stream");
         } else {
             hipLaunchKernelGGL((attn_bwd_dq_k<128, false>), gq, dim3(256), 0, st, a);
-            if (d->dK) hipLaunchKernelGGL((attn_bwd_dkdv_k<128, false>), gk, dim3(256), 0, st, a);
+            if (d->dK) launch_dkdv128(a, gk, st);
         }
     } else {
         hipLaunchKernelGGL(attn_delta_k<64>, gd, dim3(256), 0, st, a, workspace);
diff --git a/desta2.5-audio_amd/desta/_hip.py b/desta2.5-audio_amd/desta/_hip.py
--- a/desta2.5-audio_amd/desta/_hip.py
+++ b/desta2.5-audio_amd/desta/_hip.py
@@ -476,6 +476,7 @@
 lib.desta_attention_bwd_workspace_floats.restype = c_size_t
 lib.desta_attention_bwd_workspace_floats.argtypes = [i32, i32, i32]
 _attn_bwd = _sig("desta_attention_bwd", C.POINTER(AttnDesc), vp, vp)
+_attn_bwd_from = _sig("desta_attention_bwd_from", C.POINTER(AttnDesc), i32, vp, vp)
 
 
 def _elem_ptr(t, offset_elems):
@@ -568,7 +569,7 @@
 
 @_profiled(lambda d, *a, **k: "attn_bwd:" + _attn_tag(d), lambda d, *a, **k: _attn_flops(d, 2.5))
 def attention_bwd(d: AttnDesc, do, dq, dk=None, dv=None, *, do_rs=None, dq_off=0, dk_off=0, dv_off=0, dq_rs=None,
-                  dk_rs=None, dv_rs=None, do_bs=None, dq_bs=None, dk_bs=None, dv_bs=None, rope_cos_sin=None, dkv_t=None):
+                  dk_rs=None, dv_rs=None, do_bs=None, dq_bs=None, dk_bs=None, dv_bs=None, rope_cos_sin=None, dkv_t=None, grad_from=0):
     d.rope_cos_sin = p(rope_cos_sin)
     d._keep_rope = rope_cos_sin
     do_rs = do.shape[-1] if do_rs is None else do_rs
@@ -591,7 +592,10 @@
         d.dK = d.dV = 0
     ws = scratch(lib.desta_attention_bwd_workspace_floats(d.batch, d.n_q_heads, d.seq_q), do.device, "attn")
     d._keep_bwd = (do, dq, dk, dv, ws)
-    check(_attn_bwd(C.byref(d), p(ws), stream()), "desta_attention_bwd")
+    if grad_from:
+        check(_attn_bwd_from(C.byref(d), int(grad_from), p(ws), stream()), "desta_attention_bwd_from")
+    else:
+        check(_attn_bwd(C.byref(d), p(ws), stream()), "desta_attention_bwd")
 
 
 _prompt_expand = _sig("desta_prompt_expand", vp, i32, i32, i64, vp, vp, vp)
diff --git a/desta2.5-audio_amd/desta/models/modeling_desta25.py b/desta2.5-audio_amd/desta/models/modeling_desta25.py
--- a/desta2.5-audio_amd/desta/models/modeling_desta25.py
+++ b/desta2.5-audio_amd/desta/models/modeling_desta25.py
@@ -1883,12 +1883,13 @@
                     H.gemm(self.dgu[a0:], ly["wguT"], dhb[a0:], Ma, h, 2 * self.I)
                 H.rmsnorm_bwd(dhb[a0:], s["xm"][a0:], ly["n2"], s["r2"][a0:], other[a0:], dres=dx[a0:])
                 H.gemm(other[a0:], ly["woT"], self.datt[a0:], Ma, aw, h)
+            gfrom = r0 // B if self.s_major and self.skip_dead_rows else 0
             fused = getattr(self, "_rope_fused", False)
             rcs = self.cos_sin_il if fused else None
             if self.s_major:
                 H.attention_bwd(s["ad"], self.datt, self.dqkv, self.dqkv, self.dqkv, dq_off=0, dk_off=aw, dv_off=(self.hq + self.hkv) * self.hd,
                                 do_rs=B * aw, dq_rs=B * self.qkvw, dk_rs=B * self.qkvw, dv_rs=B * self.qkvw,
-                                do_bs=aw, dq_bs=self.qkvw, dk_bs=self.qkvw, dv_bs=self.qkvw, rope_cos_sin=rcs)
+                                do_bs=aw, dq_bs=self.qkvw, dk_bs=self.qkvw, dv_bs=self.qkvw, rope_cos_sin=rcs, grad_from=gfrom)
             else:
                 H.attention_bwd(s["ad"], self.datt, self.dqkv, self.dqkv, self.dqkv, dq_off=0, dk_off=aw, dv_off=(self.hq + self.hkv) * self.hd,
                                 rope_cos_sin=rcs)
diff --git a/include/desta_hip.h b/include/desta_hip.h
--- a/include/desta_hip.h
+++ b/include/desta_hip.h
@@ -183,6 +183,7 @@
 int desta_attention_fwd(const desta_attn_desc* d, void* stream);
 size_t desta_attention_bwd_workspace_floats(int batch, int n_q_heads, int seq_q);
 int desta_attention_bwd(const desta_attn_desc* d, float* workspace, void* stream);
+int desta_attention_bwd_from(const desta_attn_desc* d, int grad_from, float* workspace, void* stream);
 int desta_attention_set_concurrent_bwd(int on);
 int desta_attention_set_option(int which, int value);
 
```
